# AcrylicShrimp/omok-ai

Measured on NVIDIA B200. Metric: mcts_simulations_per_sec, higher is better.
Workload: dtype f32

## Files before the change

### include/omok_b200.h

```cpp
#ifndef OMOK_B200_H
#define OMOK_B200_H

#include <stdint.h>

#ifdef __cplusplus
extern "C" {
#endif

#if defined(__GNUC__)
#define OMK_API __attribute__((visibility("default")))
#else
#define OMK_API
#endif

#define OMK_CELLS 81
#define OMK_NONE (-1)

enum {
    OMK_OK = 0,
    OMK_ERR_INVALID = -1,
    OMK_ERR_CUDA = -2,
    OMK_ERR_CAPACITY = -3,
    OMK_ERR_STATE = -4,
    OMK_ERR_NUMERIC = -5,
};

enum {
    OMK_EVAL_NET = 0,
    OMK_EVAL_HASH = 1,
};

enum { OMK_SAMPLE_BEST = 0, OMK_SAMPLE_BOLTZMANN = 1 };
enum { OMK_TURN_MODE_PLAYER = 0, OMK_TURN_MODE_OPPONENT = 1 };

typedef struct omk_ctx omk_ctx;

OMK_API const char *omk_last_error(void);
OMK_API int32_t omk_version(void);

OMK_API int32_t omk_ctx_create(int32_t device, int32_t capacity_envs, int32_t capacity_trees, int32_t capacity_nodes,
                       uint64_t seed, omk_ctx **out);
OMK_API int32_t omk_ctx_destroy(omk_ctx *ctx);
OMK_API int32_t omk_ctx_synchronize(omk_ctx *ctx);
OMK_API void *omk_ctx_stream(omk_ctx *ctx);
OMK_API int64_t omk_ctx_launch_count(omk_ctx *ctx);
OMK_API int32_t omk_ctx_transfer_bytes(omk_ctx *ctx, int64_t *out_h2d, int64_t *out_d2h);

#define OMK_NET_TENSORS 31
OMK_API int32_t omk_net_load_params(omk_ctx *ctx, const float *const *tensors, const int64_t *lens);
OMK_API int32_t omk_net_get_params(omk_ctx *ctx, float *const *tensors, const int64_t *lens);
OMK_API int32_t omk_net_init_random(omk_ctx *ctx, uint64_t seed);
OMK_API int32_t omk_net_eval(omk_ctx *ctx, const uint8_t *boards, const uint8_t *turns, int32_t n, int32_t mode,
                     float *out_p, float *out_v);
OMK_API int32_t omk_net_eval_images(omk_ctx *ctx, const float *images, int32_t n, float *out_p, float *out_v);

OMK_API int32_t omk_train_step(omk_ctx *ctx, const float *images, const float *pi, const float *z, int32_t n, float *out_losses);
OMK_API int32_t omk_train_backward(omk_ctx *ctx, const float *images, const float *pi, const float *z, int32_t n,
                           void **out_grads_device, int64_t *out_count);
OMK_API int32_t omk_train_apply(omk_ctx *ctx, float *out_losses);
OMK_API int32_t omk_train_get_grads(omk_ctx *ctx, float *const *tensors, const int64_t *lens);
OMK_API int32_t omk_train_reset_optimizer(omk_ctx *ctx);
OMK_API int32_t omk_train_comm_unique_id(omk_ctx *ctx, uint8_t *out_id);
OMK_API int32_t omk_train_comm_init(omk_ctx *ctx, const uint8_t *id, int32_t nranks, int32_t rank);
OMK_API int32_t omk_train_comm_destroy(omk_ctx *ctx);

OMK_API int32_t omk_debug_set_fc0_mode(omk_ctx *ctx, int32_t mode);
OMK_API int32_t omk_debug_set_tower_mode(omk_ctx *ctx, int32_t mode);
OMK_API int32_t omk_debug_set_fc0_chunk(omk_ctx *ctx, int32_t k_blocks);
OMK_API int32_t omk_debug_set_fc0_balance(omk_ctx *ctx, int32_t on);
OMK_API int32_t omk_debug_tower_timing(omk_ctx *ctx, int64_t *out64);
OMK_API int32_t omk_debug_get_buffer(omk_ctx *ctx, int32_t which, float *out, int64_t count);
OMK_API int32_t omk_debug_set_lane_min_trees(omk_ctx *ctx, int32_t min_trees);

OMK_API int32_t omk_env_reset(omk_ctx *ctx, const int32_t *ids, int32_t n);
OMK_API int32_t omk_env_step(omk_ctx *ctx, const int32_t *ids, const uint8_t *actions, int32_t n, int8_t *out_status,
                     uint32_t *out_legal);
OMK_API int32_t omk_env_step_device(omk_ctx *ctx, const uint8_t *actions_device, int32_t n, int8_t *out_status_device,
                            uint32_t *out_legal_device);
OMK_API int32_t omk_env_get(omk_ctx *ctx, const int32_t *ids, int32_t n, uint8_t *out_boards, uint8_t *out_turns,
                    uint16_t *out_legal_counts);
OMK_API int32_t omk_env_set(omk_ctx *ctx, const int32_t *ids, int32_t n, const uint8_t *boards, const uint8_t *turns);
OMK_API int32_t omk_env_encode(omk_ctx *ctx, const int32_t *ids, int32_t n, int32_t mode, float *out);
OMK_API int32_t omk_env_random_playout(omk_ctx *ctx, int32_t n, int32_t plies, uint8_t *out_actions, int8_t *out_status);

OMK_API int32_t omk_pool_new_games(omk_ctx *ctx, const int32_t *ids, int32_t n, const uint32_t *streams, int32_t evaluator);
OMK_API int32_t omk_pool_search(omk_ctx *ctx, const int32_t *ids, int32_t n, int32_t count, int32_t batch_size,
                        float epsilon, float alpha, int32_t evaluator);
OMK_API int32_t omk_search_set_virtual_loss(omk_ctx *ctx, int32_t enabled);
OMK_API int32_t omk_pool_sample(omk_ctx *ctx, const int32_t *ids, int32_t n, const uint8_t *modes,
                        const float *temperatures, int32_t *out_actions, float *out_policy);
OMK_API int32_t omk_pool_policy(omk_ctx *ctx, const int32_t *ids, int32_t n, float *out_policy, uint8_t *out_valid);
OMK_API int32_t omk_pool_ensure_action(omk_ctx *ctx, const int32_t *ids, const int32_t *actions, int32_t n,
                               int32_t evaluator);
OMK_API int32_t omk_pool_play(omk_ctx *ctx, const int32_t *ids, const int32_t *actions, int32_t n, int8_t *out_status);
OMK_API int32_t omk_pool_get_env(omk_ctx *ctx, int32_t id, uint8_t *out_board, uint8_t *out_turn,
                         uint16_t *out_legal_count);
OMK_API int32_t omk_pool_get_envs(omk_ctx *ctx, const int32_t *ids, int32_t n, uint8_t *out_boards, uint8_t *out_turns,
                          uint16_t *out_legal_counts, int8_t *out_status);
OMK_API int32_t omk_pool_root_stats(omk_ctx *ctx, int32_t id, uint64_t *out_n, float *out_w, float *out_p,
                            int32_t *out_status, float *out_policy);
OMK_API int32_t omk_pool_root_children(omk_ctx *ctx, int32_t id, int32_t *out_actions, uint64_t *out_n, float *out_w,
                               float *out_p, int32_t *out_len);
OMK_API int32_t omk_pool_tree_info(omk_ctx *ctx, int32_t id, int32_t *out_nodes, uint32_t *out_rng_counter);

enum {
    OMK_K_TOWER = 0,
    OMK_K_FC0 = 1,
    OMK_K_FC1 = 2,
    OMK_K_HEADS = 3,
    OMK_K_HASH = 4,
    OMK_K_SELECT = 5,
    OMK_K_APPLY = 6,
    OMK_K_MOVE = 7,
    OMK_K_COUNT = 8
};

typedef struct {
    int32_t n_games;
    int32_t count;
    int32_t batch_size;
    float epsilon;
    float alpha;
    float temperature;
    int32_t temperature_threshold;
    int32_t evaluator;
} omk_selfplay_config;

typedef struct {
    int64_t simulations;
    int64_t positions;
    int64_t nn_evals;
    int64_t games_finished;
    int64_t h2d_bytes, d2h_bytes;
    float gpu_ms;
    float kind_ms[OMK_K_COUNT];
    int64_t kind_launches[OMK_K_COUNT];
} omk_selfplay_stats;

OMK_API int32_t omk_selfplay_begin(omk_ctx *ctx, const omk_selfplay_config *cfg);
OMK_API int32_t omk_selfplay_run(omk_ctx *ctx, int32_t plies, int32_t profile, uint8_t *out_boards, float *out_policy,
                         int8_t *out_status, int32_t *out_actions, omk_selfplay_stats *stats);

OMK_API int32_t omk_replay_reset(omk_ctx *ctx, int64_t capacity);
OMK_API int32_t omk_replay_info(omk_ctx *ctx, int64_t *out_len, int64_t *out_rows_added, int64_t *out_episodes);
OMK_API int32_t omk_replay_get(omk_ctx *ctx, const int64_t *rows, int32_t n, uint8_t *out_boards, uint8_t *out_turns,
                       float *out_policy, float *out_z);
OMK_API int32_t omk_train_replay(omk_ctx *ctx, uint64_t seed, int64_t first_step, int32_t steps, int32_t n, float *out_losses,
                         int64_t *out_rows);

OMK_API int32_t omk_naive_move(omk_ctx *ctx, const uint8_t *boards, const uint8_t *turns, int32_t n, uint64_t seed,
                               const uint32_t *streams, int32_t *out_actions, uint8_t *out_forced);
OMK_API int32_t omk_eval_naive(omk_ctx *ctx, int32_t episodes, int32_t first_tree, int32_t count, int32_t batch_size, float epsilon,
                               float alpha, int32_t evaluator, uint64_t seed, int32_t *out_result, int8_t *out_moves,
                               int8_t *out_status, int64_t *out_stats, float *out_gpu_ms);

// ... 13 lines not shown
```

### omok-ai_b200/binding.py

```python
from __future__ import annotations

import ctypes as C
import os
import re

import numpy as np

CELLS = 81
NONE = -1
EVAL_NET, EVAL_HASH = 0, 1
SAMPLE_BEST, SAMPLE_BOLTZMANN = 0, 1

_HERE = os.path.dirname(os.path.abspath(__file__))
_ROOT = os.path.dirname(_HERE)

NET_LENS = [384, 128] + [4096, 32, 288, 1024, 32, 4096, 128] * 3 + [10368 * 512, 512, 512 * 512, 512, 512, 1, 512 * 81, 81]
NET_SHAPES = (
    [(1, 1, 3, 128), (128,)]
    + [(1, 1, 128, 32), (32,), (3, 3, 32, 1), (1, 1, 32, 32), (32,), (1, 1, 32, 128), (128,)] * 3
    + [(10368, 512), (512,), (512, 512), (512,), (512, 1), (1,), (512, 81), (81,)]
)


class OmkError(RuntimeError):
# ... 4 lines not shown

class SelfPlayConfig(C.Structure):
    _fields_ = [
        ("n_games", C.c_int32),
        ("count", C.c_int32),
        ("batch_size", C.c_int32),
        ("epsilon", C.c_float),
        ("alpha", C.c_float),
        ("temperature", C.c_float),
        ("temperature_threshold", C.c_int32),
        ("evaluator", C.c_int32),
    ]


class SelfPlayStats(C.Structure):
    _fields_ = [
        ("simulations", C.c_int64),
        ("positions", C.c_int64),
        ("nn_evals", C.c_int64),
        ("games_finished", C.c_int64),
        ("h2d_bytes", C.c_int64),
        ("d2h_bytes", C.c_int64),
        ("gpu_ms", C.c_float),
        ("kind_ms", C.c_float * 8),
        ("kind_launches", C.c_int64 * 8),
    ]

    KINDS = ("tower", "fc0", "fc1", "heads", "hash", "select_expand", "apply", "move")

    def by_kind(self):
        return {k: (float(self.kind_ms[i]), int(self.kind_launches[i])) for i, k in enumerate(self.KINDS)}


def lib_path() -> str:
    return os.path.join(_HERE, "libomok_b200.so")


def declared_symbols() -> list[str]:
    text = open(os.path.join(_ROOT, "include", "omok_b200.h")).read()
    return sorted(set(re.findall(r"OMK_API[^;(]*?\b(omk_\w+)\s*\(", text)))


_lib = None


def load_library():
    global _lib
    if _lib is not None:
        return _lib
    path = lib_path()
    if not os.path.exists(path):
        raise OmkError(-2, f"{path} is missing: run __graft_entry__.build() (there is no CPU fallback)")
    L = C.CDLL(path)
    P = C.POINTER
    i32, i64, u64, f32, vp = C.c_int32, C.c_int64, C.c_uint64, C.c_float, C.c_void_p
    L.omk_last_error.restype = C.c_char_p
    L.omk_version.restype = i32
    L.omk_ctx_create.argtypes = [i32, i32, i32, i32, u64, P(vp)]
    L.omk_ctx_destroy.argtypes = [vp]
    L.omk_ctx_synchronize.argtypes = [vp]
    L.omk_ctx_stream.argtypes = [vp]
    L.omk_ctx_stream.restype = vp
    L.omk_ctx_launch_count.argtypes = [vp]
    L.omk_ctx_launch_count.restype = i64
    L.omk_ctx_transfer_bytes.argtypes = [vp, P(i64), P(i64)]
    L.omk_net_load_params.argtypes = [vp, P(vp), P(i64)]
    L.omk_net_get_params.argtypes = [vp, P(vp), P(i64)]
    L.omk_net_init_random.argtypes = [vp, u64]
    L.omk_net_eval.argtypes = [vp, vp, vp, i32, i32, vp, vp]
    L.omk_net_eval_images.argtypes = [vp, vp, i32, vp, vp]
    L.omk_train_step.argtypes = [vp, vp, vp, vp, i32, vp]
    L.omk_train_backward.argtypes = [vp, vp, vp, vp, i32, P(vp), P(i64)]
    L.omk_train_apply.argtypes = [vp, vp]
    L.omk_train_get_grads.argtypes = [vp, P(vp), P(i64)]
    L.omk_train_reset_optimizer.argtypes = [vp]
    L.omk_train_comm_unique_id.argtypes = [vp, vp]
    L.omk_train_comm_init.argtypes = [vp, vp, i32, i32]
    L.omk_train_comm_destroy.argtypes = [vp]
    L.omk_debug_set_fc0_mode.argtypes = [vp, i32]
    L.omk_debug_set_tower_mode.argtypes = [vp, i32]
    L.omk_debug_set_fc0_chunk.argtypes = [vp, i32]
    L.omk_debug_set_fc0_balance.argtypes = [vp, i32]
    L.omk_debug_set_lane_min_trees.argtypes = [vp, i32]
    L.omk_debug_get_buffer.argtypes = [vp, i32, vp, i64]
    L.omk_debug_tower_timing.argtypes = [vp, vp]
    L.omk_env_reset.argtypes = [vp, vp, i32]
    L.omk_env_step.argtypes = [vp, vp, vp, i32, vp, vp]
    L.omk_env_step_device.argtypes = [vp, vp, i32, vp, vp]
    L.omk_env_get.argtypes = [vp, vp, i32, vp, vp, vp]
    L.omk_env_set.argtypes = [vp, vp, i32, vp, vp]
    L.omk_env_encode.argtypes = [vp, vp, i32, i32, vp]
    L.omk_env_random_playout.argtypes = [vp, i32, i32, vp, vp]
    L.omk_pool_new_games.argtypes = [vp, vp, i32, vp, i32]
    L.omk_pool_search.argtypes = [vp, vp, i32, i32, i32, f32, f32, i32]
    L.omk_search_set_virtual_loss.argtypes = [vp, i32]
    L.omk_pool_sample.argtypes = [vp, vp, i32, vp, vp, vp, vp]
    L.omk_pool_policy.argtypes = [vp, vp, i32, vp, vp]
    L.omk_pool_ensure_action.argtypes = [vp, vp, vp, i32, i32]
    L.omk_pool_play.argtypes = [vp, vp, vp, i32, vp]
    L.omk_pool_get_env.argtypes = [vp, i32, vp, vp, vp]
    L.omk_pool_get_envs.argtypes = [vp, vp, i32, vp, vp, vp, vp]
    L.omk_pool_root_stats.argtypes = [vp, i32, vp, vp, vp, vp, vp]
    L.omk_pool_root_children.argtypes = [vp, i32, vp, vp, vp, vp, vp]
    L.omk_pool_tree_info.argtypes = [vp, i32, vp, vp]
    L.omk_selfplay_begin.argtypes = [vp, P(SelfPlayConfig)]
    L.omk_selfplay_run.argtypes = [vp, i32, i32, vp, vp, vp, vp, P(SelfPlayStats)]
    L.omk_replay_reset.argtypes = [vp, i64]
    L.omk_replay_info.argtypes = [vp, P(i64), P(i64), P(i64)]
    L.omk_replay_get.argtypes = [vp, vp, i32, vp, vp, vp, vp]
    L.omk_train_replay.argtypes = [vp, u64, i64, i32, i32, vp, vp]
    L.omk_naive_move.argtypes = [vp, vp, vp, i32, u64, vp, vp, vp]
    L.omk_eval_naive.argtypes = [vp, i32, i32, i32, i32, f32, f32, i32, u64, vp, vp, vp, vp, P(f32)]
    L.omk_opponent_load_params.argtypes = [vp, P(vp), P(i64)]
    L.omk_opponent_from_net.argtypes = [vp]
    L.omk_opponent_eval.argtypes = [vp, vp, vp, i32, i32, vp, vp]
    L.omk_match.argtypes = [vp, i32, i32, i32, i32, f32, f32, i32, vp, vp, vp, vp, P(f32)]
    for name in declared_symbols():
        fn = getattr(L, name)
        if name not in ("omk_last_error", "omk_ctx_stream", "omk_ctx_launch_count"):
            fn.restype = i32
    _lib = L
    return L


def _ptr(a):
    return None if a is None else a.ctypes.data_as(C.c_void_p)


def _ids(ids):
    return None if ids is None else np.ascontiguousarray(ids, dtype=np.int32)


class Context:

    def __init__(self, device: int = 0, capacity_envs: int = 0, capacity_trees: int = 0, capacity_nodes: int = 4096,
                 seed: int = 0):
        self.L = load_library()
        h = C.c_void_p()
        self.h = None
        self._check(self.L.omk_ctx_create(device, capacity_envs, capacity_trees, capacity_nodes, seed, C.byref(h)))
        self.h = h
        self.capacity_envs, self.capacity_trees, self.capacity_nodes = capacity_envs, capacity_trees, capacity_nodes
        self.seed = seed

    def _check(self, rc: int):
        if rc != 0:
            raise OmkError(rc, self.L.omk_last_error().decode())

    def close(self):
        if self.h is not None:
            self.L.omk_ctx_destroy(self.h)
            self.h = None

    def __del__(self):
        try:
            self.close()
        except Exception:
            pass

    def synchronize(self):
        self._check(self.L.omk_ctx_synchronize(self.h))

    @property
    def stream(self) -> int:
        return int(self.L.omk_ctx_stream(self.h) or 0)

# ... 22 lines not shown

    def net_init_random(self, seed: int = 0):
        self._check(self.L.omk_net_init_random(self.h, seed))

    def net_eval(self, boards, turns, mode: int = 0, want_v: bool = True):
        boards = np.ascontiguousarray(boards, dtype=np.uint8).reshape(-1, CELLS)
        turns = np.ascontiguousarray(turns, dtype=np.uint8).reshape(-1)
        n = boards.shape[0]
        p = np.zeros((n, CELLS), dtype=np.float32)
        v = np.zeros(n, dtype=np.float32) if want_v else None
        self._check(self.L.omk_net_eval(self.h, _ptr(boards), _ptr(turns), n, mode, _ptr(p), _ptr(v)))
        return p, v

    def net_eval_images(self, images, want_v: bool = True):
        images = np.ascontiguousarray(images, dtype=np.float32).reshape(-1, 243)
        n = images.shape[0]
        p = np.zeros((n, CELLS), dtype=np.float32)
        v = np.zeros(n, dtype=np.float32) if want_v else None
        self._check(self.L.omk_net_eval_images(self.h, _ptr(images), n, _ptr(p), _ptr(v)))
        return p, v

    @staticmethod
    def _batch(images, pi, z):
        images = np.ascontiguousarray(images, dtype=np.float32).reshape(-1, 243)
        n = images.shape[0]
        pi = np.ascontiguousarray(pi, dtype=np.float32).reshape(n, CELLS)
        z = np.ascontiguousarray(z, dtype=np.float32).reshape(n)
        return images, pi, z, n

    def train_step(self, images, pi, z):
        images, pi, z, n = self._batch(images, pi, z)
        out = np.zeros(3, dtype=np.float32)
        self._check(self.L.omk_train_step(self.h, _ptr(images), _ptr(pi), _ptr(z), n, _ptr(out)))
        return float(out[0]), float(out[1]), float(out[2])

    def train_backward(self, images, pi, z):
        images, pi, z, n = self._batch(images, pi, z)
        ptr, cnt = C.c_void_p(), C.c_int64()
        self._check(self.L.omk_train_backward(self.h, _ptr(images), _ptr(pi), _ptr(z), n, C.byref(ptr), C.byref(cnt)))
        return int(ptr.value or 0), int(cnt.value)

    def train_apply(self):
        out = np.zeros(3, dtype=np.float32)
        self._check(self.L.omk_train_apply(self.h, _ptr(out)))
        return float(out[0]), float(out[1]), float(out[2])

    def train_get_grads(self):
        arrs = [np.zeros(n, dtype=np.float32) for n in NET_LENS]
        ptrs = (C.c_void_p * 31)(*[a.ctypes.data for a in arrs])
        lens = (C.c_int64 * 31)(*NET_LENS)
        self._check(self.L.omk_train_get_grads(self.h, ptrs, lens))
        return [a.reshape(s) for a, s in zip(arrs, NET_SHAPES)]

    def train_reset_optimizer(self):
        self._check(self.L.omk_train_reset_optimizer(self.h))

    def train_comm_unique_id(self) -> bytes:
        buf = np.zeros(128, dtype=np.uint8)
        self._check(self.L.omk_train_comm_unique_id(self.h, _ptr(buf)))
        return buf.tobytes()

    def train_comm_init(self, unique_id: bytes, nranks: int, rank: int):
        buf = np.frombuffer(unique_id, dtype=np.uint8).copy()
        self._check(self.L.omk_train_comm_init(self.h, _ptr(buf), nranks, rank))

    def train_comm_destroy(self):
        self._check(self.L.omk_train_comm_destroy(self.h))

    def debug_set_fc0_mode(self, mode: int):
        self._check(self.L.omk_debug_set_fc0_mode(self.h, mode))

    def debug_set_tower_mode(self, mode: int):
        self._check(self.L.omk_debug_set_tower_mode(self.h, mode))

    def debug_set_fc0_balance(self, on: bool):
        self._check(self.L.omk_debug_set_fc0_balance(self.h, 1 if on else 0))

    def debug_set_fc0_chunk(self, k_blocks: int):
        self._check(self.L.omk_debug_set_fc0_chunk(self.h, k_blocks))

    def debug_set_lane_min_trees(self, min_trees: int):
        self._check(self.L.omk_debug_set_lane_min_trees(self.h, min_trees))

    def debug_tower_timing(self):
        out = np.zeros(64, dtype=np.int64)
        self._check(self.L.omk_debug_tower_timing(self.h, _ptr(out)))
        return out

    def debug_get_buffer(self, which: int, count: int):
        out = np.zeros(count, dtype=np.float32)
        self._check(self.L.omk_debug_get_buffer(self.h, which, _ptr(out), count))
        return out

    def env_reset(self, ids=None, n=None):
        ids = _ids(ids)
        n = len(ids) if ids is not None else n
        self._check(self.L.omk_env_reset(self.h, _ptr(ids), n))

    def env_step(self, actions, ids=None, want_legal: bool = True):
        actions = np.ascontiguousarray(actions, dtype=np.uint8)
        ids = _ids(ids)
        n = actions.size
        status = np.zeros(n, dtype=np.int8)
        legal = np.zeros((n, 3), dtype=np.uint32) if want_legal else None
        self._check(self.L.omk_env_step(self.h, _ptr(ids), _ptr(actions), n, _ptr(status), _ptr(legal)))
        return status, legal

    def env_step_device(self, actions_dev: int, n: int, status_dev: int, legal_dev: int):
        self._check(self.L.omk_env_step_device(self.h, actions_dev, n, status_dev, legal_dev))

    def env_get(self, ids=None, n=None):
        ids = _ids(ids)
        n = len(ids) if ids is not None else n
        boards = np.zeros((n, CELLS), dtype=np.uint8)
        turns = np.zeros(n, dtype=np.uint8)
        legal = np.zeros(n, dtype=np.uint16)
        self._check(self.L.omk_env_get(self.h, _ptr(ids), n, _ptr(boards), _ptr(turns), _ptr(legal)))
        return boards, turns, legal

    def env_set(self, boards, turns, ids=None):
        boards = np.ascontiguousarray(boards, dtype=np.uint8).reshape(-1, CELLS)
        turns = np.ascontiguousarray(turns, dtype=np.uint8).reshape(-1)
        ids = _ids(ids)
        self._check(self.L.omk_env_set(self.h, _ptr(ids), boards.shape[0], _ptr(boards), _ptr(turns)))

    def env_encode(self, ids=None, n=None, mode: int = 0):
        ids = _ids(ids)
        n = len(ids) if ids is not None else n
        out = np.zeros((n, 243), dtype=np.float32)
        self._check(self.L.omk_env_encode(self.h, _ptr(ids), n, mode, _ptr(out)))
        return out

    def env_random_playout(self, n: int, plies: int, trace: bool = True):
        actions = np.zeros((plies, n), dtype=np.uint8) if trace else None
        status = np.zeros((plies, n), dtype=np.int8) if trace else None
        self._check(self.L.omk_env_random_playout(self.h, n, plies, _ptr(actions), _ptr(status)))
        return actions, status

    def pool_new_games(self, ids=None, n=None, streams=None, evaluator: int = EVAL_NET):
        ids = _ids(ids)
        n = len(ids) if ids is not None else n
        streams = None if streams is None else np.ascontiguousarray(streams, dtype=np.uint32)
        self._check(self.L.omk_pool_new_games(self.h, _ptr(ids), n, _ptr(streams), evaluator))

    def pool_search(self, ids=None, n=None, count=800, batch_size=16, epsilon=0.25, alpha=0.03, evaluator: int = EVAL_NET):
        ids = _ids(ids)
        n = len(ids) if ids is not None else n
        self._check(self.L.omk_pool_search(self.h, _ptr(ids), n, count, batch_size, epsilon, alpha, evaluator))

    def search_set_virtual_loss(self, enabled: bool):
        self._check(self.L.omk_search_set_virtual_loss(self.h, 1 if enabled else 0))

    def pool_sample(self, ids=None, n=None, modes=None, temperatures=None):
        ids = _ids(ids)
        n = len(ids) if ids is not None else n
        modes = None if modes is None else np.ascontiguousarray(modes, dtype=np.uint8)
        temperatures = None if temperatures is None else np.ascontiguousarray(temperatures, dtype=np.float32)
        actions = np.zeros(n, dtype=np.int32)
        policy = np.zeros((n, CELLS), dtype=np.float32)
        self._check(self.L.omk_pool_sample(self.h, _ptr(ids), n, _ptr(modes), _ptr(temperatures), _ptr(actions), _ptr(policy)))
        return actions, policy

    def pool_policy(self, ids=None, n=None):
        ids = _ids(ids)
        n = len(ids) if ids is not None else n
        policy = np.zeros((n, CELLS), dtype=np.float32)
# ... 156 lines not shown
```

### omok-ai_b200/csrc/fc_f16.cu

```cuda
#include <cstdio>
#include <cstdlib>
#include <cuda.h>

#include "omk_internal.h"
#include "tc_ptx.cuh"

namespace omk {

using namespace tc;

constexpr int F_BM = 128, F_BN = 256, F_BK = 64;
constexpr int F_N = 512;
constexpr int F_K0 = 10368, F_K1 = 512;
constexpr int F_A_BYTES = F_BM * F_BK * 2;
#ifndef OMK_F_CHUNK1
#define OMK_F_CHUNK1 1
#endif
#ifndef OMK_F_CHUNKH
#define OMK_F_CHUNKH 1
#endif
constexpr int F_SPLITK_KB = 9;
constexpr int F_CHUNK0 = 9, F_CHUNK0_FINE = 3;
constexpr int F_CHUNK1 = OMK_F_CHUNK1;
constexpr int F_CHUNKH = OMK_F_CHUNKH;
constexpr int kSplitKMaxRows = 2048;

struct FcBal {
    int full;
    int helpers;
    int m, tail;
    int mains;
    float4 *partial;
    uint32_t *flags;
};
constexpr int F_BAL_TAIL_MAX = 4;
constexpr size_t F_BAL_UNIT_F4 = 2 * 8 * 32 * 32;
__device__ __forceinline__ uint32_t ld_acquire_u32(const uint32_t *p) {
    uint32_t v;
    asm volatile("ld.acquire.gpu.global.u32 %0, [%1];" : "=r"(v) : "l"(p) : "memory");
    return v;
}

template <bool PAIR, int BN>
struct FcCfg {
    static constexpr int kStages = PAIR ? 3 : 2;
    static constexpr int kBRows = PAIR ? BN / 2 : BN;
    static constexpr int kBBytes = kBRows * F_BK * 2;
    static constexpr int kStageBytes = 2 * F_A_BYTES + 2 * kBBytes;
    static constexpr int kSmemBytes = kStages * kStageBytes + 1024 + 1024;
    static constexpr uint32_t kIdesc = idesc_f16(PAIR ? 256 : 128, BN);
    static constexpr int kDrainWarps = 4 * (BN / 128);
    static constexpr int kThreads = 64 + 32 * kDrainWarps;
    static constexpr uint32_t kTmemCols = 2 * BN;
};

template <int K, int CHUNK, bool PAIR, int BN = 256, bool HEADS = false, bool SPLITK = false>
__global__ void __launch_bounds__((FcCfg<PAIR, BN>::kThreads), 1)
    k_fc16(const __grid_constant__ CUtensorMap map_a_hi, const __grid_constant__ CUtensorMap map_a_lo,
           const __grid_constant__ CUtensorMap map_b_hi, const __grid_constant__ CUtensorMap map_b_lo,
           const float *__restrict__ bias, const float *__restrict__ inv_scale_p, float *__restrict__ C,
           __half *__restrict__ C_hi, __half *__restrict__ C_lo, const uint32_t *n_req, int max_rows,
           float *__restrict__ P_out = nullptr, float *__restrict__ V_out = nullptr, uint32_t *dev_error = nullptr,
           const FcBal bal = FcBal{}) {
    using Cfg = FcCfg<PAIR, BN>;
    static_assert(!HEADS || (BN == 128 && !PAIR), "the heads epilogue needs a whole logit row per thread");
    constexpr int CG = PAIR ? 2 : 1;
    static_assert(K % F_BK == 0 && (K / F_BK) % CHUNK == 0, "chunking must tile K");
    static_assert(!SPLITK || (!PAIR && !HEADS), "split-K is the one-CTA fc0 variant");
    constexpr int NKB = SPLITK ? F_SPLITK_KB : K / F_BK;
    static_assert(!SPLITK || (F_SPLITK_KB % CHUNK == 0 && (K / F_BK) % F_SPLITK_KB == 0), "split-K groups must tile K");
    constexpr int NCHUNK = NKB / CHUNK;
    const int kb_base = SPLITK ? (int)blockIdx.z * F_SPLITK_KB : 0;
    extern __shared__ uint8_t smem_raw[];
    const int rows = (int)min(*n_req, (uint32_t)max_rows);
    uint32_t rank = 0;
    int m0, n0;
    [[maybe_unused]] int role = 0, n_seq = NCHUNK, u0 = 0;
    [[maybe_unused]] int tile = 0;
    if constexpr (PAIR) {
        rank = cluster_rank();
        const int cid = blockIdx.x >> 1;
        tile = cid;
        if (cid >= bal.full && bal.helpers > 0) {
            if (cid < bal.full + bal.helpers) {
                role = 2;
                const int units = bal.mains * bal.tail, h = cid - bal.full;
                const int per = (units + bal.helpers - 1) / bal.helpers;
                u0 = h * per;
                n_seq = max(0, min(units, u0 + per) - u0);
            } else {
                role = 1;
                tile = cid - bal.helpers;
                n_seq = bal.m;
            }
        }
        const int pair = tile >> 1;
        m0 = pair * 256 + (int)rank * F_BM;
        n0 = (tile & 1) * BN;
        if (role != 2 && pair * 256 >= rows) return;
    } else {
        m0 = blockIdx.y * F_BM;
        n0 = blockIdx.x * BN;
        if (m0 >= rows) return;
    }
    const bool leader = rank == 0;

    const uint32_t base = (smem_u32(smem_raw) + 1023u) & ~1023u;
    const uint32_t bars = base + Cfg::kStages * Cfg::kStageBytes;
    const uint32_t full0 = bars, empty0 = bars + 8 * Cfg::kStages, tmem_full0 = bars + 16 * Cfg::kStages,
                   tmem_empty0 = tmem_full0 + 16, tmem_slot = tmem_empty0 + 16;
    const int warp = threadIdx.x >> 5, lane = threadIdx.x & 31;

    if (warp == 0 && lane == 0) {
        prefetch_map(&map_a_hi);
        prefetch_map(&map_a_lo);
        prefetch_map(&map_b_hi);
        prefetch_map(&map_b_lo);
        for (int s = 0; s < Cfg::kStages; ++s) {
            mbar_init(full0 + 8 * s, 1);
            mbar_init(empty0 + 8 * s, 1);
        }
        for (int b = 0; b < 2; ++b) {
            mbar_init(tmem_full0 + 8 * b, 1);
            mbar_init(tmem_empty0 + 8 * b, (PAIR ? 2 : 1) * Cfg::kDrainWarps);
        }
        mbar_fence_init();
    }
    if (warp == 1) tmem_alloc<CG>(tmem_slot, Cfg::kTmemCols);
    fence_before();
    __syncthreads();
    if constexpr (PAIR) cluster_sync_all();
    fence_after();
    uint32_t tmem_base;
    asm volatile("ld.shared.u32 %0, [%1];" : "=r"(tmem_base) : "r"(tmem_slot));

    if (warp == 0) {
        if (lane == 0) {
            if constexpr (PAIR) {
                int it = 0;
                for (int i = 0; i < n_seq; ++i) {
                    int ch = i, mm = m0, nn = n0;
                    if (role == 2) {
                        const int u = u0 + i, tl = bal.full + u / bal.tail;
                        ch = bal.m + u % bal.tail;
                        mm = (tl >> 1) * 256 + (int)rank * F_BM;
                        nn = (tl & 1) * BN;
                        if ((tl >> 1) * 256 >= rows) continue;
                    }
                    for (int kc = 0; kc < CHUNK; ++kc, ++it) {
                        const int kb = ch * CHUNK + kc, s = it % Cfg::kStages;
                        const uint32_t ph = (uint32_t)(it / Cfg::kStages) & 1u;
                        mbar_wait(empty0 + 8 * s, ph ^ 1u);
                        const uint32_t st = base + s * Cfg::kStageBytes;
                        const uint32_t lbar = mapa(full0 + 8 * s, 0);
                        if (leader) mbar_expect_tx(full0 + 8 * s, 2 * Cfg::kStageBytes);
                        tma_load_2d_2sm(st, &map_a_hi, lbar, kb * F_BK, mm);
                        tma_load_2d_2sm(st + F_A_BYTES, &map_a_lo, lbar, kb * F_BK, mm);
                        tma_load_2d_2sm(st + 2 * F_A_BYTES, &map_b_hi, lbar, kb * F_BK, nn + (int)rank * 128);
                        tma_load_2d_2sm(st + 2 * F_A_BYTES + Cfg::kBBytes, &map_b_lo, lbar, kb * F_BK, nn + (int)rank * 128);
                    }
                }
            }
            for (int kb = 0; kb < (PAIR ? 0 : NKB); ++kb) {
                const int s = kb % Cfg::kStages;
                const uint32_t ph = (uint32_t)(kb / Cfg::kStages) & 1u;
                mbar_wait(empty0 + 8 * s, ph ^ 1u);
                const uint32_t st = base + s * Cfg::kStageBytes;
                if constexpr (PAIR) {
                } else {
                    const uint32_t bar = full0 + 8 * s;
                    mbar_expect_tx(bar, Cfg::kStageBytes);
                    tma_load_2d(st, &map_a_hi, bar, (kb_base + kb) * F_BK, m0);
                    tma_load_2d(st + F_A_BYTES, &map_a_lo, bar, (kb_base + kb) * F_BK, m0);
                    tma_load_2d(st + 2 * F_A_BYTES, &map_b_hi, bar, (kb_base + kb) * F_BK, n0);
                    tma_load_2d(st + 2 * F_A_BYTES + Cfg::kBBytes, &map_b_lo, bar, (kb_base + kb) * F_BK, n0);
                }
            }
        }
    } else if (warp == 1) {
        if (leader && lane == 0) {
            for (int i = 0, ci = 0, it = 0; i < n_seq; ++i) {
                if constexpr (PAIR) {
                    if (role == 2 && ((bal.full + (u0 + i) / bal.tail) >> 1) * 256 >= rows) continue;
                }
                const int buf = ci & 1;
                const uint32_t use = (uint32_t)(ci >> 1);
                ++ci;
                mbar_wait(tmem_empty0 + 8 * buf, (use & 1u) ^ 1u);
                fence_after();
                const uint32_t tmem_acc = tmem_base + (uint32_t)(buf * BN);
                for (int kc = 0; kc < CHUNK; ++kc, ++it) {
                    const int s = it % Cfg::kStages;
                    const uint32_t ph = (uint32_t)(it / Cfg::kStages) & 1u;
                    mbar_wait(full0 + 8 * s, ph);
                    fence_after();
                    const uint32_t st = base + s * Cfg::kStageBytes;
                    const uint64_t a_hi = desc_sw128(st), a_lo = desc_sw128(st + F_A_BYTES);
                    const uint64_t b_hi = desc_sw128(st + 2 * F_A_BYTES), b_lo = desc_sw128(st + 2 * F_A_BYTES + Cfg::kBBytes);
#pragma unroll
                    for (int k = 0; k < F_BK / 16; ++k) {
                        const uint64_t adv = (uint64_t)((k * 32) >> 4);
                        umma_f16_ss<CG>(tmem_acc, a_lo + adv, b_hi + adv, Cfg::kIdesc, (kc | k) != 0 ? 1u : 0u);
                        umma_f16_ss<CG>(tmem_acc, a_hi + adv, b_lo + adv, Cfg::kIdesc, 1u);
                        umma_f16_ss<CG>(tmem_acc, a_hi + adv, b_hi + adv, Cfg::kIdesc, 1u);
                    }
                    if constexpr (PAIR) umma_commit_2sm(empty0 + 8 * s); else umma_commit(empty0 + 8 * s);
                }
                if constexpr (PAIR) umma_commit_2sm(tmem_full0 + 8 * buf); else umma_commit(tmem_full0 + 8 * buf);
            }
        }
    } else {
        const int q = warp & 3, half = (warp - 2) >> 2;
        float acc[128];
#pragma unroll
        for (int j = 0; j < 128; ++j) acc[j] = 0.0f;
        for (int ch = 0, ci = 0; ch < n_seq; ++ch) {
            [[maybe_unused]] float4 *unit_dst = nullptr;
            [[maybe_unused]] int unit_main = 0;
            if constexpr (PAIR) {
                if (role == 2) {
                    const int u = u0 + ch;
                    unit_main = u / bal.tail;
                    if (((bal.full + unit_main) >> 1) * 256 >= rows) continue;
                    unit_dst = bal.partial + (((size_t)u * 2 + rank) * 8 + (size_t)(warp - 2)) * 1024 + lane;
                }
            }
            const int buf = ci & 1;
            const uint32_t use = (uint32_t)(ci >> 1);
            ++ci;
            mbar_wait(tmem_full0 + 8 * buf, use & 1u);
            fence_after();
#pragma unroll
            for (int c = 0; c < 128; c += 32) {
                float v[32];
                tmem_ld32(tmem_base + ((uint32_t)(q * 32) << 16) + (uint32_t)(buf * BN + half * 128 + c), v);
                tmem_wait_ld();
                if (PAIR && role == 2) {
#pragma unroll
                    for (int j = 0; j < 32; j += 4) unit_dst[(size_t)((c + j) >> 2) * 32] = make_float4(v[j], v[j + 1], v[j + 2], v[j + 3]);
                } else {
#pragma unroll
                    for (int j = 0; j < 32; ++j) acc[c + j] += v[j];
                }
            }
            fence_before();
            __syncwarp();
            if (lane == 0) {
                if constexpr (PAIR) mbar_arrive_cluster(mapa(tmem_empty0 + 8 * buf, 0)); else mbar_arrive(tmem_empty0 + 8 * buf);
            }
            if constexpr (PAIR) {
                if (role == 2) {
                    __threadfence();
                    __syncwarp();
                    if (lane == 0) atomicAdd(bal.flags + unit_main, 1u);
                }
            }
            if constexpr (SPLITK) {
                const int prow = m0 + q * 32 + lane;
// ... 21 lines not shown
                    for (int c4 = 0; c4 < 32; ++c4) {
                        const float4 v = __ldcg(src + (size_t)c4 * 32);
                        acc[4 * c4 + 0] += v.x; acc[4 * c4 + 1] += v.y; acc[4 * c4 + 2] += v.z; acc[4 * c4 + 3] += v.w;
                    }
                }
                __syncwarp();
                if (lane == 0 && atomicAdd(bal.flags + 128 + k, 1u) == 15u) {
                    atomicExch(bal.flags + k, 0u);
                    atomicExch(bal.flags + 128 + k, 0u);
                }
            }
        }
        const int row = m0 + q * 32 + lane;
        const size_t coff = (size_t)row * F_N + n0 + half * 128;
        const float *brow = bias + n0 + half * 128;
        const float inv_scale = *inv_scale_p;
        if constexpr (SPLITK) {
        } else if constexpr (HEADS) {
            if (row < rows) {
                float mx = -INFINITY;
#pragma unroll
                for (int j = 0; j < kCells; ++j) {
                    acc[j] = fmaf(acc[j], inv_scale, brow[j]);
                    mx = fmaxf(mx, acc[j]);
                }
                float sum = 0.0f;
#pragma unroll
                for (int j = 0; j < kCells; ++j) {
                    acc[j] = expf(acc[j] - mx);
                    sum += acc[j];
                }
                const float inv = 1.0f / sum;
                const float vlogit = fmaf(acc[kCells], inv_scale, brow[kCells]);
                if (!(sum >= 1.0f && sum < INFINITY) || !(fabsf(vlogit) < INFINITY)) atomicOr(dev_error, 2u);
                float *prow = P_out + (size_t)row * kRow;
#pragma unroll
                for (int j = 0; j < 80; j += 4)
                    *reinterpret_cast<float4 *>(prow + j) = make_float4(acc[j] * inv, acc[j + 1] * inv, acc[j + 2] * inv, acc[j + 3] * inv);
                prow[80] = acc[80] * inv;
                V_out[row] = tanhf(vlogit);
            }
        } else if (row < rows && role != 2) {
#pragma unroll
            for (int j = 0; j < 128; j += 8) {
                float o[8];
#pragma unroll
                for (int i = 0; i < 8; i += 4) {
                    const float4 b = *reinterpret_cast<const float4 *>(brow + j + i);
                    o[i + 0] = fmaf(acc[j + i + 0], inv_scale, b.x);
                    o[i + 1] = fmaf(acc[j + i + 1], inv_scale, b.y);
                    o[i + 2] = fmaf(acc[j + i + 2], inv_scale, b.z);
                    o[i + 3] = fmaf(acc[j + i + 3], inv_scale, b.w);
                }
#pragma unroll
                for (int i = 0; i < 8; ++i) o[i] = fmaxf(o[i], 0.2f * o[i]);
                if (C) {
                    *reinterpret_cast<float4 *>(C + coff + j) = make_float4(o[0], o[1], o[2], o[3]);
                    *reinterpret_cast<float4 *>(C + coff + j + 4) = make_float4(o[4], o[5], o[6], o[7]);
                }
                if (C_hi) {
                    uint4 h, l;
                    split2_f16(o[0], o[1], h.x, l.x);
                    split2_f16(o[2], o[3], h.y, l.y);
                    split2_f16(o[4], o[5], h.z, l.z);
                    split2_f16(o[6], o[7], h.w, l.w);
                    *reinterpret_cast<uint4 *>(C_hi + coff + j) = h;
                    *reinterpret_cast<uint4 *>(C_lo + coff + j) = l;
                }
            }
        }
    }
    fence_before();
    __syncthreads();
    if constexpr (PAIR) cluster_sync_all();
    if (warp == 1) {
        fence_after();
        tmem_dealloc<CG>(tmem_base, Cfg::kTmemCols);
    }
}

__global__ void k_fc0_reduce(const float *__restrict__ partial, int nchunks, int ws_rows, const float *__restrict__ bias,
                             const float *__restrict__ inv_scale_p, __half *__restrict__ C_hi, __half *__restrict__ C_lo,
                             const uint32_t *n_req, int max_rows) {
    const int rows = (int)min(*n_req, (uint32_t)max_rows);
    const int idx = blockIdx.x * blockDim.x + threadIdx.x;
    const int row = idx >> 6, j = (idx & 63) * 8;
    if (row >= rows) return;
    float acc[8];
#pragma unroll
    for (int i = 0; i < 8; ++i) acc[i] = 0.0f;
    for (int z0 = 0; z0 < nchunks; z0 += 6) {
        float4 a[6], b[6];
#pragma unroll
        for (int i = 0; i < 6; ++i) {
            const int z = min(z0 + i, nchunks - 1);
            const float *p = partial + ((size_t)z * ws_rows + row) * F_N + j;
            a[i] = *reinterpret_cast<const float4 *>(p);
            b[i] = *reinterpret_cast<const float4 *>(p + 4);
        }
#pragma unroll
        for (int i = 0; i < 6; ++i) {
            if (z0 + i >= nchunks) break;
            acc[0] += a[i].x; acc[1] += a[i].y; acc[2] += a[i].z; acc[3] += a[i].w;
            acc[4] += b[i].x; acc[5] += b[i].y; acc[6] += b[i].z; acc[7] += b[i].w;
        }
    }
    const float inv_scale = *inv_scale_p;
    float o[8];
#pragma unroll
    for (int i = 0; i < 8; ++i) {
        o[i] = fmaf(acc[i], inv_scale, bias[j + i]);
        o[i] = fmaxf(o[i], 0.2f * o[i]);
    }
    uint4 h, l;
    split2_f16(o[0], o[1], h.x, l.x);
    split2_f16(o[2], o[3], h.y, l.y);
    split2_f16(o[4], o[5], h.z, l.z);
    split2_f16(o[6], o[7], h.w, l.w);
    *reinterpret_cast<uint4 *>(C_hi + (size_t)row * F_N + j) = h;
    *reinterpret_cast<uint4 *>(C_lo + (size_t)row * F_N + j) = l;
}

__global__ void k_absmax_bits(const float *__restrict__ w, long long n, uint32_t *out) {
    uint32_t m = 0;
    for (long long i = (long long)blockIdx.x * blockDim.x + threadIdx.x; i < n; i += (long long)gridDim.x * blockDim.x)
        m = max(m, __float_as_uint(w[i]) & 0x7FFFFFFFu);
#pragma unroll
    for (int off = 16; off > 0; off >>= 1) m = max(m, __shfl_xor_sync(0xffffffffu, m, off));
    if ((threadIdx.x & 31) == 0 && m) atomicMax(out, m);
}

__global__ void k_fc16_split_weights(const float *__restrict__ W, const uint32_t *absmax_bits, __half *__restrict__ hi,
                                     __half *__restrict__ lo, float *inv_scale, int K, int N) {
    __shared__ float tile[32][33];
    const float scale = f16_split_scale(*absmax_bits);
    if (blockIdx.x == 0 && blockIdx.y == 0 && threadIdx.x == 0) *inv_scale = 1.0f / scale;
    const int k0 = blockIdx.x * 32, n0 = blockIdx.y * 32;
    const int tx = threadIdx.x & 31, ty = threadIdx.x >> 5;
    for (int r = ty; r < 32; r += 8) tile[r][tx] = W[(size_t)(k0 + r) * N + n0 + tx];
    __syncthreads();
    for (int r = ty; r < 32; r += 8) {
        const float x = tile[tx][r] * scale;
        const __half h = __float2half_rn(x);
        hi[(size_t)(n0 + r) * K + k0 + tx] = h;
        lo[(size_t)(n0 + r) * K + k0 + tx] = __float2half_rn(x - __half2float(h));
    }
}

__global__ void k_f32_to_split16(const float *__restrict__ x, __half *__restrict__ hi, __half *__restrict__ lo, long long n) {
    for (long long i = (long long)blockIdx.x * blockDim.x + threadIdx.x; i < n; i += (long long)gridDim.x * blockDim.x) {
        const __half h = __float2half_rn(x[i]);
        hi[i] = h;
        lo[i] = __float2half_rn(x[i] - __half2float(h));
    }
}
__global__ void k_split16_to_f32(const __half *__restrict__ hi, const __half *__restrict__ lo, float *__restrict__ x, long long n) {
    for (long long i = (long long)blockIdx.x * blockDim.x + threadIdx.x; i < n; i += (long long)gridDim.x * blockDim.x)
        x[i] = __half2float(hi[i]) + __half2float(lo[i]);
}
void launch_f32_to_split16(omk_ctx *c, const float *x, __half *hi, __half *lo, long long n) {
    k_f32_to_split16<<<1184, 256, 0, c->stream>>>(x, hi, lo, n);
    c->launches++;
}
void launch_split16_to_f32(omk_ctx *c, const __half *hi, const __half *lo, float *x, long long n) {
    k_split16_to_f32<<<1184, 256, 0, c->stream>>>(hi, lo, x, n);
    c->launches++;
// ... 32 lines not shown
    const cuuint32_t box[3] = {32, 32, 1};
    const cuuint32_t estr[3] = {1, 1, 1};
    return fn(map, CU_TENSOR_MAP_DATA_TYPE_FLOAT16, 3, ptr, dims, strides, box, estr, CU_TENSOR_MAP_INTERLEAVE_NONE,
              CU_TENSOR_MAP_SWIZZLE_64B, CU_TENSOR_MAP_L2_PROMOTION_NONE, CU_TENSOR_MAP_FLOAT_OOB_FILL_NONE) == CUDA_SUCCESS;
}

struct Fc16State {
    int pair_slots = 0;
};
void Fc16StateFree::operator()(Fc16State *s) const { delete s; }

static Fc16State *state16_of(omk_ctx *c) {
    if (!c->fc16_state) c->fc16_state.reset(new Fc16State());
    return c->fc16_state.get();
}

bool fc16_prepare_weights(omk_ctx *c) {
    NetWeights &w = *c->model;
    if (!w.fc0_wt_h16) {
        FcImages f;
        if (f.fc0_wt_h16.alloc((size_t)F_K0 * F_N) != cudaSuccess || f.fc0_wt_l16.alloc((size_t)F_K0 * F_N) != cudaSuccess ||
            f.fc1_wt_h16.alloc((size_t)F_K1 * F_N) != cudaSuccess || f.fc1_wt_l16.alloc((size_t)F_K1 * F_N) != cudaSuccess ||
            f.heads_wt_h16.alloc((size_t)F_K1 * 128) != cudaSuccess || f.heads_wt_l16.alloc((size_t)F_K1 * 128) != cudaSuccess ||
            f.fc_inv_scale.alloc(3) != cudaSuccess || f.fc_absmax.alloc(3) != cudaSuccess)
            return false;
        static_cast<FcImages &>(w) = std::move(f);
    }
    cudaMemsetAsync(w.fc_absmax, 0, sizeof(uint32_t) * 3, c->stream);
    k_absmax_bits<<<592, 256, 0, c->stream>>>(w.t[23], (long long)F_K0 * F_N, w.fc_absmax);
    k_absmax_bits<<<148, 256, 0, c->stream>>>(w.t[25], (long long)F_K1 * F_N, w.fc_absmax + 1);
    k_absmax_bits<<<64, 256, 0, c->stream>>>(w.heads_w, (long long)F_K1 * 128, w.fc_absmax + 2);
    k_fc16_split_weights<<<dim3(F_K0 / 32, F_N / 32), 256, 0, c->stream>>>(w.t[23], w.fc_absmax, w.fc0_wt_h16, w.fc0_wt_l16,
                                                                           w.fc_inv_scale, F_K0, F_N);
    k_fc16_split_weights<<<dim3(F_K1 / 32, F_N / 32), 256, 0, c->stream>>>(w.t[25], w.fc_absmax + 1, w.fc1_wt_h16, w.fc1_wt_l16,
                                                                           w.fc_inv_scale + 1, F_K1, F_N);
    k_fc16_split_weights<<<dim3(F_K1 / 32, 128 / 32), 256, 0, c->stream>>>(w.heads_w, w.fc_absmax + 2, w.heads_wt_h16, w.heads_wt_l16,
                                                                         w.fc_inv_scale + 2, F_K1, 128);
    c->launches += 6;
    if (!encode_map16(&w.map0_b_hi, w.fc0_wt_h16, F_N, 128, F_K0)) return false;
    if (!encode_map16(&w.map0_b_lo, w.fc0_wt_l16, F_N, 128, F_K0)) return false;
    if (!encode_map16(&w.map0s_b_hi, w.fc0_wt_h16, F_N, F_BN, F_K0)) return false;
    if (!encode_map16(&w.map0s_b_lo, w.fc0_wt_l16, F_N, F_BN, F_K0)) return false;
    if (!encode_map16(&w.map1_b_hi, w.fc1_wt_h16, F_N, F_BN, F_K1)) return false;
    if (!encode_map16(&w.map1_b_lo, w.fc1_wt_l16, F_N, F_BN, F_K1)) return false;
    if (!encode_map16(&w.map2_b_hi, w.heads_wt_h16, 128, 128, F_K1)) return false;
    if (!encode_map16(&w.map2_b_lo, w.heads_wt_l16, 128, 128, F_K1)) return false;
    w.weights_ready = true;
    return true;
}

bool fc16_encode_act_maps(Activations &a) {
    ActMaps &m = a.maps;
    const uint64_t rows = (uint64_t)a.act_rows;
    return encode_map16(&m.map0_a_hi, a.act0_h16, rows, F_BM, F_K0) && encode_map16(&m.map0_a_lo, a.act0_l16, rows, F_BM, F_K0) &&
           encode_map16(&m.map1_a_hi, a.act1_h16, rows, F_BM, F_K1) && encode_map16(&m.map1_a_lo, a.act1_l16, rows, F_BM, F_K1) &&
           encode_map16(&m.map2_a_hi, a.act2_h16, rows, F_BM, F_K1) && encode_map16(&m.map2_a_lo, a.act2_l16, rows, F_BM, F_K1) &&
           encode_map_tower_store(&m.tower_st_hi, a.act0_h16, rows) && encode_map_tower_store(&m.tower_st_lo, a.act0_l16, rows);
}

static bool check_launch(const char *what) {
    const cudaError_t le = cudaPeekAtLastError();
    if (le == cudaSuccess) return true;
    fprintf(stderr, "omok_b200: %s launch failed: %s\n", what, cudaGetErrorString(le));
    return false;
}

bool launch_fc0_f16(omk_ctx *c, int rows_bound) {
    const NetWeights &m = *c->model;
    const ActMaps *am = m.weights_ready ? &c->ws.maps : nullptr;
    if (!am) return false;
    const bool fine = c->fc0_chunk == F_CHUNK0_FINE;
    static const int splitk_env = getenv("OMK_FC0_SPLITK_MAX") ? atoi(getenv("OMK_FC0_SPLITK_MAX")) : -1;
    const int splitk_max = splitk_env >= 0 ? splitk_env : (fine ? 1024 : kSplitKMaxRows);
    if (rows_bound <= splitk_max) {
        const int kChunks = F_K0 / F_BK / (fine ? F_CHUNK0_FINE : F_CHUNK0);
        const int mt = (rows_bound + F_BM - 1) / F_BM, ws_rows = mt * F_BM;
        if (c->ws.splitk_partial.grow(c->stream, (size_t)kChunks * ws_rows * F_N) != cudaSuccess) return false;
        float *partial = c->ws.splitk_partial;
        static const int narrow_env = getenv("OMK_FC0_SPLITK_NARROW") ? atoi(getenv("OMK_FC0_SPLITK_NARROW")) : -1;
        if (mt <= (narrow_env >= 0 ? narrow_env : 2)) {
            using Cfg = FcCfg<false, 128>;
            auto sk = fine ? k_fc16<F_K0, F_CHUNK0_FINE, false, 128, false, true> : k_fc16<F_K0, F_CHUNK0, false, 128, false, true>;
            cudaFuncSetAttribute(sk, cudaFuncAttributeMaxDynamicSharedMemorySize, Cfg::kSmemBytes);
            sk<<<dim3(F_N / 128, mt, F_K0 / F_BK / F_SPLITK_KB), Cfg::kThreads, Cfg::kSmemBytes, c->stream>>>(
                am->map0_a_hi, am->map0_a_lo, m.map0_b_hi, m.map0_b_lo, m.t[24], m.fc_inv_scale, partial, nullptr,
                nullptr, c->ws.n_req, rows_bound, nullptr, nullptr, nullptr, FcBal{});
        } else {
            using Cfg = FcCfg<false, 256>;
            auto sk = fine ? k_fc16<F_K0, F_CHUNK0_FINE, false, 256, false, true> : k_fc16<F_K0, F_CHUNK0, false, 256, false, true>;
            cudaFuncSetAttribute(sk, cudaFuncAttributeMaxDynamicSharedMemorySize, Cfg::kSmemBytes);
            sk<<<dim3(F_N / F_BN, mt, F_K0 / F_BK / F_SPLITK_KB), Cfg::kThreads, Cfg::kSmemBytes, c->stream>>>(
                am->map0_a_hi, am->map0_a_lo, m.map0s_b_hi, m.map0s_b_lo, m.t[24], m.fc_inv_scale, partial, nullptr,
                nullptr, c->ws.n_req, rows_bound, nullptr, nullptr, nullptr, FcBal{});
        }
        k_fc0_reduce<<<(rows_bound * 64 + 255) / 256, 256, 0, c->stream>>>(partial, kChunks, ws_rows, m.t[24],
                                                                            m.fc_inv_scale, c->ws.act1_h16, c->ws.act1_l16,
                                                                            c->ws.n_req, rows_bound);
        c->launches += 2;
        return check_launch("fc0 (fp16 split, split-K)");
    }
    auto kern = fine ? k_fc16<F_K0, F_CHUNK0_FINE, true> : k_fc16<F_K0, F_CHUNK0, true>;
    cudaFuncSetAttribute(kern, cudaFuncAttributeMaxDynamicSharedMemorySize, FcCfg<true, 256>::kSmemBytes);
    const int pairs = (rows_bound + 255) / 256;
    cudaLaunchConfig_t cfg{};
    cfg.gridDim = dim3(2 * (F_N / F_BN) * pairs, 1);
    cfg.blockDim = dim3(FcCfg<true, 256>::kThreads);
    cfg.dynamicSmemBytes = FcCfg<true, 256>::kSmemBytes;
    cfg.stream = c->stream;
    cudaLaunchAttribute attr[1];
    attr[0].id = cudaLaunchAttributeClusterDimension;
    attr[0].val.clusterDim.x = 2;
    attr[0].val.clusterDim.y = 1;
    attr[0].val.clusterDim.z = 1;
    cfg.attrs = attr;
    cfg.numAttrs = 1;
    const float *bias_p = m.t[24];
    const float *inv_p = m.fc_inv_scale;
    float *c_f32 = nullptr;
    __half *c_hi = c->ws.act1_h16, *c_lo = c->ws.act1_l16;
    const uint32_t *nreq_p = c->ws.n_req;
    float *no_p = nullptr, *no_v = nullptr;
    uint32_t *no_err = nullptr;
    FcBal bal{};
    if (!fine && c->fc0_balance) {
        Fc16State *st = state16_of(c);
        if (st->pair_slots == 0) {
            int n = 0;
            if (cudaOccupancyMaxActiveClusters(&n, kern, &cfg) != cudaSuccess) { cudaGetLastError(); n = 0; }
            st->pair_slots = n > 0 ? n : -1;
        }
        const int P = st->pair_slots, T = (F_N / F_BN) * pairs, NC = F_K0 / F_BK / F_CHUNK0;
        const int R = P > 0 ? T % P : 0, H = P - R;
        if (R > 0 && R <= 128 && H > 0) {
            int tail = 0;
            for (int t = 1; t <= F_BAL_TAIL_MAX; ++t)
                if ((R * t + H - 1) / H + 1 <= NC - t) tail = t;
            if (tail > 0) {
                const int units = R * tail;
                bool ok = true;
                Workspace &w = c->ws;
                if (!w.bal_flags)
                    ok = w.bal_flags.alloc(256) == cudaSuccess && cudaMemsetAsync(w.bal_flags, 0, w.bal_flags.bytes(), c->stream) == cudaSuccess;
                if (!ok || w.bal_partial.grow(c->stream, F_BAL_UNIT_F4 * (size_t)units) != cudaSuccess) return false;
                bal.full = T - R;
                bal.helpers = H;
                bal.mains = R;
                bal.tail = tail;
                bal.m = NC - tail;
                bal.partial = w.bal_partial;
                bal.flags = w.bal_flags;
                cfg.gridDim = dim3(2 * (T + H), 1);
            }
        }
    }
    const cudaError_t e = cudaLaunchKernelEx(&cfg, kern, am->map0_a_hi, am->map0_a_lo, m.map0_b_hi, m.map0_b_lo, bias_p, inv_p, c_f32,
                                             c_hi, c_lo, nreq_p, rows_bound, no_p, no_v, no_err, bal);
    if (e != cudaSuccess) fprintf(stderr, "omok_b200: cudaLaunchKernelEx(k_fc16 pair): %s\n", cudaGetErrorString(e));
    c->launches++;
    return e == cudaSuccess && check_launch("fc0 (fp16 split)");
}

bool launch_fc1_f16(omk_ctx *c, int rows_bound) {
    const NetWeights &m = *c->model;
    const ActMaps *am = m.weights_ready ? &c->ws.maps : nullptr;
    if (!am) return false;
    using Cfg = FcCfg<false, 256>;
    auto kern = k_fc16<F_K1, F_CHUNK1, false>;
    cudaFuncSetAttribute(kern, cudaFuncAttributeMaxDynamicSharedMemorySize, Cfg::kSmemBytes);
    const int mt = (rows_bound + F_BM - 1) / F_BM;
    kern<<<dim3(F_N / F_BN, mt), Cfg::kThreads, Cfg::kSmemBytes, c->stream>>>(
        am->map1_a_hi, am->map1_a_lo, m.map1_b_hi, m.map1_b_lo, m.t[26], m.fc_inv_scale + 1, nullptr, c->ws.act2_h16,
        c->ws.act2_l16, c->ws.n_req, rows_bound, nullptr, nullptr, nullptr, FcBal{});
    c->launches++;
    return check_launch("fc1 (fp16 split)");
}

bool launch_heads_f16(omk_ctx *c, int rows_bound) {
    const NetWeights &m = *c->model;
    const ActMaps *am = m.weights_ready ? &c->ws.maps : nullptr;
    if (!am) return false;
    using Cfg = FcCfg<false, 128>;
    auto kern = k_fc16<F_K1, F_CHUNKH, false, 128, true>;
    cudaFuncSetAttribute(kern, cudaFuncAttributeMaxDynamicSharedMemorySize, Cfg::kSmemBytes);
    const int mt = (rows_bound + F_BM - 1) / F_BM;
    kern<<<dim3(1, mt), Cfg::kThreads, Cfg::kSmemBytes, c->stream>>>(
        am->map2_a_hi, am->map2_a_lo, m.map2_b_hi, m.map2_b_lo, m.heads_b, m.fc_inv_scale + 2, nullptr, nullptr, nullptr,
        c->ws.n_req, rows_bound, c->ws.P, c->ws.V, c->dev_error, FcBal{});
    c->launches++;
    return check_launch("heads (fp16 split)");
}

}
```

### omok-ai_b200/csrc/omk_api.cu

```cuda
#include <cstdio>
#include <cstdlib>
#include <cstring>
#include <string>
#include <vector>

#include <utility>

#include "omk_internal.h"

using namespace omk;

static thread_local std::string g_err;
static int32_t fail(int32_t code, const std::string &msg) {
    g_err = msg;
    return code;
}
#define CK(call)                                                                                        \
    do {                                                                                                \
        cudaError_t e__ = (call);                                                                       \
        if (e__ != cudaSuccess)                                                                         \
            return fail(OMK_ERR_CUDA, std::string(#call) + ": " + cudaGetErrorString(e__));             \
    } while (0)
#define CKV(call)                                                                                       \
    do {                                                                                                \
// ... 471 lines not shown
extern "C" int32_t omk_train_apply(omk_ctx *c, float *out_losses) {
    CK(cudaSetDevice(c->device));
    if (c->train_n < 1) return fail(OMK_ERR_STATE, "omk_train_backward has not produced a gradient");
    if (const char *e = train_apply_step(c)) return fail(OMK_ERR_CUDA, std::string("omk_train_apply: ") + e);
    c->net_pack_dirty = true;
    float l[3] = {0, 0, 0};
    if (const char *e = train_report_losses(c, c->train_n, l)) return fail(OMK_ERR_CUDA, std::string("omk_train_apply: ") + e);
    c->train_n = 0;
    if (!(l[2] == l[2]) || l[2] > 3.0e38f) return fail(OMK_ERR_NUMERIC, "the training loss is not finite");
    if (out_losses) memcpy(out_losses, l, sizeof l);
    return OMK_OK;
}

extern "C" int32_t omk_train_step(omk_ctx *c, const float *images, const float *pi, const float *z, int32_t n, float *out_losses) {
    int32_t rc = train_backward_impl(c, images, pi, z, n, nullptr, nullptr, false);
    if (rc) return rc;
    return omk_train_apply(c, out_losses);
}

extern "C" int32_t omk_train_get_grads(omk_ctx *c, float *const *tensors, const int64_t *lens) {
    CK(cudaSetDevice(c->device));
    const float *g = train_grad_buffer(c);
    if (!g) return fail(OMK_ERR_STATE, "omk_train_backward has not run");
    long long off = 0;
    for (int i = 0; i < kNetTensors; ++i) {
        if (!tensors[i] || lens[i] != kLens[i]) return fail(OMK_ERR_INVALID, "bad tensor length");
        CK(copy_d2h(c, tensors[i], g + off, sizeof(float) * (size_t)kLens[i], c->stream));
        off += kLens[i];
    }
    CK(cudaStreamSynchronize(c->stream));
    return OMK_OK;
}

extern "C" int32_t omk_train_reset_optimizer(omk_ctx *c) {
    CK(cudaSetDevice(c->device));
    train_reset_optimizer(c);
    CK(cudaStreamSynchronize(c->stream));
    return OMK_OK;
}

extern "C" int32_t omk_train_comm_unique_id(omk_ctx *c, uint8_t *out_id) {
    if (!out_id) return fail(OMK_ERR_INVALID, "out_id is NULL");
    if (const char *e = train_comm_unique_id(c, out_id)) return fail(OMK_ERR_STATE, std::string("NCCL: ") + e);
    return OMK_OK;
}
extern "C" int32_t omk_train_comm_init(omk_ctx *c, const uint8_t *id, int32_t nranks, int32_t rank) {
    CK(cudaSetDevice(c->device));
    if (!id || nranks < 1 || rank < 0 || rank >= nranks) return fail(OMK_ERR_INVALID, "bad communicator arguments");
    if (const char *e = train_comm_init(c, id, nranks, rank)) return fail(OMK_ERR_STATE, std::string("NCCL: ") + e);
    return OMK_OK;
}
extern "C" int32_t omk_train_comm_destroy(omk_ctx *c) {
    CK(cudaSetDevice(c->device));
    train_comm_destroy(c);
    return OMK_OK;
}

extern "C" int32_t omk_debug_set_fc0_mode(omk_ctx *c, int32_t mode) {
    if (mode != 0 && mode != 1) return fail(OMK_ERR_INVALID, "fc0 mode must be 1 (tcgen05 3xFP16) or 0 (fp32 CUDA cores, A/B check)");
    c->fc0_mode = mode;
    return OMK_OK;
}
extern "C" int32_t omk_debug_set_tower_mode(omk_ctx *c, int32_t mode) {
    if (mode != 0 && mode != 1) return fail(OMK_ERR_INVALID, "tower mode must be 1 (tcgen05 3xFP16) or 0 (fp32 CUDA cores, A/B check)");
    c->tower_mode = mode;
    return OMK_OK;
}
extern "C" int32_t omk_debug_set_fc0_balance(omk_ctx *c, int32_t on) {
    if (on != 0 && on != 1) return fail(OMK_ERR_INVALID, "fc0 balance must be 0 or 1");
    c->fc0_balance = on;
    return OMK_OK;
}
extern "C" int32_t omk_debug_set_fc0_chunk(omk_ctx *c, int32_t k_blocks) {
    if (k_blocks != 3 && k_blocks != 9) return fail(OMK_ERR_INVALID, "fc0 chunk must be 9 (default) or 3 (finer accumulation)");
    CK(cudaStreamSynchronize(c->stream));
    c->fc0_chunk = k_blocks;
    return OMK_OK;
}
extern "C" int32_t omk_debug_set_lane_min_trees(omk_ctx *c, int32_t min_trees) {
    if (min_trees < 0) return fail(OMK_ERR_INVALID, "min_trees < 0");
    c->lane_min_trees = min_trees;
    return OMK_OK;
}
extern "C" int32_t omk_debug_tower_timing(omk_ctx *c, int64_t *out64) {
    CK(cudaSetDevice(c->device));
    CK(cudaStreamSynchronize(c->stream));
    tower16_read_timing(reinterpret_cast<long long *>(out64));
    return OMK_OK;
}
extern "C" int32_t omk_debug_get_buffer(omk_ctx *c, int32_t which, float *out, int64_t count) {
    CK(cudaSetDevice(c->device));
    if (which >= 8 && which <= 10) {
        if (!out || count < 0) return fail(OMK_ERR_INVALID, "bad buffer");
        const __half *hi = which == 8 ? c->ws.act0_h16 : which == 9 ? c->ws.act1_h16 : c->ws.act2_h16;
        const __half *lo = which == 8 ? c->ws.act0_l16 : which == 9 ? c->ws.act1_l16 : c->ws.act2_l16;
        if (!hi || !lo) return fail(OMK_ERR_STATE, "the tensor-core activation buffers do not exist yet (no network call so far)");
        float *tmp = nullptr;
        SCRATCH(0, (size_t)(count > 0 ? count : 1), tmp);
        launch_split16_to_f32(c, hi, lo, tmp, count);
        CK(copy_d2h(c, out, tmp, sizeof(float) * (size_t)count, c->stream));
        CK(cudaStreamSynchronize(c->stream));
        return OMK_OK;
    }
    const float *src = which == 0 ? c->ws.act0 : which == 1 ? c->ws.act1 : which == 2 ? c->ws.act2 : which == 3 ? c->ws.logits.get() : nullptr;
    if (!src || !out || count < 0) return fail(OMK_ERR_INVALID, "bad buffer id");
    CK(copy_d2h(c, out, src, sizeof(float) * (size_t)count, c->stream));
    CK(cudaStreamSynchronize(c->stream));
    return OMK_OK;
}

extern "C" int32_t omk_env_reset(omk_ctx *c, const int32_t *ids, int32_t n) {
    CK(cudaSetDevice(c->device));
    const int32_t *d_ids;
    int32_t rc = stage_ids(c, ids, n, &d_ids, c->cap_envs);
    if (rc) return rc;
    launch_env_reset(c, d_ids, n);
    CK(cudaStreamSynchronize(c->stream));
    return OMK_OK;
}

extern "C" int32_t omk_env_step(omk_ctx *c, const int32_t *ids, const uint8_t *actions, int32_t n, int8_t *out_status,
                                uint32_t *out_legal) {
    CK(cudaSetDevice(c->device));
    if (!actions) return fail(OMK_ERR_INVALID, "actions is NULL");
    const int32_t *d_ids;
    int32_t rc = stage_ids(c, ids, n, &d_ids, c->cap_envs);
    if (rc) return rc;
    if (n == 0) return OMK_OK;
    uint8_t *d_act = nullptr;
    int8_t *d_st = nullptr;
    uint32_t *d_legal = nullptr;
    SCRATCH(0, (size_t)n, d_act);
    SCRATCH(1, (size_t)n, d_st);
    if (out_legal) SCRATCH(2, 3 * (size_t)n, d_legal);
    CK(copy_h2d(c, d_act, actions, (size_t)n, c->stream));
    launch_env_step(c, d_ids, d_act, n, d_st, d_legal);
    if (out_status) CK(copy_d2h(c, out_status, d_st, (size_t)n, c->stream));
    if (out_legal) CK(copy_d2h(c, out_legal, d_legal, sizeof(uint32_t) * 3 * (size_t)n, c->stream));
    CK(cudaStreamSynchronize(c->stream));
    CK(cudaGetLastError());
    return OMK_OK;
}

extern "C" int32_t omk_env_step_device(omk_ctx *c, const uint8_t *actions_device, int32_t n, int8_t *out_status_device,
                                       uint32_t *out_legal_device) {
    if (n < 0 || n > c->cap_envs) return fail(OMK_ERR_INVALID, "n exceeds capacity_envs");
    launch_env_step(c, nullptr, actions_device, n, out_status_device, out_legal_device);
    return OMK_OK;
}

extern "C" int32_t omk_env_get(omk_ctx *c, const int32_t *ids, int32_t n, uint8_t *out_boards, uint8_t *out_turns,
                               uint16_t *out_legal_counts) {
    CK(cudaSetDevice(c->device));
    const int32_t *d_ids;
    int32_t rc = stage_ids(c, ids, n, &d_ids, c->cap_envs);
    if (rc) return rc;
    if (n == 0) return OMK_OK;
    uint8_t *d_b = nullptr, *d_t = nullptr;
    uint16_t *d_l = nullptr;
    SCRATCH(0, (size_t)n * kCells, d_b);
    SCRATCH(1, (size_t)n, d_t);
    SCRATCH(2, (size_t)n, d_l);
    launch_env_get(c, d_ids, n, d_b, d_t, d_l);
    if (out_boards) CK(copy_d2h(c, out_boards, d_b, (size_t)n * kCells, c->stream));
    if (out_turns) CK(copy_d2h(c, out_turns, d_t, (size_t)n, c->stream));
    if (out_legal_counts) CK(copy_d2h(c, out_legal_counts, d_l, sizeof(uint16_t) * (size_t)n, c->stream));
// ... 1009 lines not shown
```

### omok-ai_b200/csrc/omk_internal.h

```cpp
#pragma once
#include <cstdint>
#include <memory>
#include <utility>
#include <vector>
#include <cuda.h>
#include <cuda_fp16.h>
#include <cuda_runtime.h>

#include "../../include/omok_b200.h"
#include "omk_device.cuh"

namespace omk {

constexpr int kMaxBatchPerTree = 64;
constexpr int kNetTensors = 31;

enum ApplyMode { kApplySearch = 0, kApplyNewGame = 1, kApplyEnsure = 2 };

struct DeviceMem {
    static cudaError_t alloc(void **p, size_t bytes) { return cudaMalloc(p, bytes); }
    static void release(void *p) { cudaFree(p); }
};
struct PinnedMem {
    static cudaError_t alloc(void **p, size_t bytes) { return cudaHostAlloc(p, bytes, cudaHostAllocDefault); }
// ... 115 lines not shown
    uint8_t *turns;
    float *pi;
    float *z;
    long long cap;
};
struct ReplayStore {
    Buf<uint8_t> boards, turns;
    Buf<float> pi, z;
    long long cap = 0;
    ReplayRing view() const { return {boards, turns, pi, z, cap}; }
};
struct ReplayCounters {
    long long added, len, episodes;
    uint32_t done, pad;
};
struct ReplayStaging {
    int games = 0;
    Buf<uint8_t> boards;
    Buf<float> pi;
    Buf<int32_t> len;
};
struct Replay {
    ReplayStore ring;
    Buf<ReplayCounters> counters;
    long long added = 0, len = 0, episodes = 0;
    ReplayStaging stage;
    cudaStream_t stream = nullptr;
    cudaEvent_t ev_commit = nullptr;
};

struct Fc16State;
struct TrainState;
struct Fc16StateFree { void operator()(Fc16State *s) const; };
struct TrainStateFree { void operator()(TrainState *t) const; };

}

struct omk_prof_span {
    cudaEvent_t a, b;
    int kind;
};

struct omk_ctx {
    ~omk_ctx();
    int device = 0;
    int prof_level = 0;
    std::vector<omk_prof_span> prof_spans;
    std::vector<cudaEvent_t> prof_pool;
    int n_sms = 0;
    int cap_envs = 0, cap_trees = 0, cap_nodes = 0;
    uint64_t seed = 0;
    cudaStream_t stream = nullptr;
    int64_t launches = 0;
    int64_t h2d_bytes = 0, d2h_bytes = 0;
    cudaStream_t lane1_stream = nullptr;
    omk::Workspace lane1_ws;
    cudaEvent_t lane_fork = nullptr, lane_join = nullptr;
    int lane_min_trees = 768;
    omk::Buf<uint8_t> scratch[3];
    std::vector<uint8_t> id_seen;
    int id_base = 0;

    omk::Buf<omk::EnvRec> envs;
    omk::Buf<omk::TreeHdr> tree_hdrs;
    omk::Buf<uint8_t> tree_nodes;
    omk::Buf<uint16_t> remap;
    omk::Buf<uint32_t> dev_error;
    omk::Buf<unsigned long long> dev_sims;

    omk::NetWeights net;
    omk::NetWeights opp;
    omk::NetWeights *model = &net;
    omk::Workspace ws;
    int virtual_loss = 0;
    int fc0_balance = 0;
    int fc0_chunk = 9;
    int fc0_mode = 1;
    std::unique_ptr<omk::Fc16State, omk::Fc16StateFree> fc16_state;
    int tower16_pairs = 0;
    std::unique_ptr<omk::TrainState, omk::TrainStateFree> train_state;
    int train_n = 0;
    bool net_pack_dirty = false;
    int tower_mode = 1;

    omk_selfplay_config sp_cfg{};
    bool sp_active = false;
    omk::Buf<int32_t> sp_ply;
    omk::Buf<uint8_t> sp_buf;
    static constexpr int kSpRing = 4;
    omk::Buf<uint8_t> sp_ring_dev;
    omk::PinnedBuf<uint8_t> sp_ring_host;
    size_t sp_ring_slot_bytes = 0;
    cudaStream_t sp_copy_stream = nullptr;
    cudaEvent_t sp_ev_rec[kSpRing][2] = {}, sp_ev_copy[kSpRing] = {};
    omk::Replay rp;
    omk::Buf<uint8_t> eval_buf;
    cudaEvent_t ev0 = nullptr, ev1 = nullptr;
};

namespace omk {

void launch_env_reset(omk_ctx *c, const int32_t *ids_dev, int n);
void launch_env_step(omk_ctx *c, const int32_t *ids_dev, const uint8_t *actions_dev, int n, int8_t *status_dev,
                     uint32_t *legal_dev);
void launch_env_get(omk_ctx *c, const int32_t *ids_dev, int n, uint8_t *boards_dev, uint8_t *turns_dev,
                    uint16_t *legal_dev);
void launch_env_set(omk_ctx *c, const int32_t *ids_dev, int n, const uint8_t *boards_dev, const uint8_t *turns_dev);
void launch_env_encode(omk_ctx *c, const int32_t *ids_dev, int n, int mode, float *out_dev);
void launch_env_playout(omk_ctx *c, int n, int plies, uint8_t *actions_dev, int8_t *status_dev);
void launch_pack_boards(omk_ctx *c, const uint8_t *boards_dev, const uint8_t *turns_dev, int n, int mode);

void launch_new_games(omk_ctx *c, const int32_t *ids_dev, int n, const uint32_t *streams_dev,
                      const int8_t *only_if_terminal, const float *root_policy);
void launch_root_noise(omk_ctx *c, const int32_t *ids_dev, int n, float epsilon, float alpha);
void launch_select_expand(omk_ctx *c, const int32_t *ids_dev, int n, int batch);
void launch_apply(omk_ctx *c, const int32_t *ids_dev, int n, int mode);
void launch_sample(omk_ctx *c, const int32_t *ids_dev, int n, const uint8_t *modes_dev, const float *temps_dev,
                   int32_t *actions_dev, float *policy_dev, uint8_t *valid_dev);
void launch_ensure_prepare(omk_ctx *c, const int32_t *ids_dev, const int32_t *actions_dev, int n);
void launch_play(omk_ctx *c, const int32_t *ids_dev, const int32_t *actions_dev, int n, int8_t *status_dev);
void launch_root_children(omk_ctx *c, int tree, int32_t *actions_dev, unsigned long long *n_dev, float *w_dev,
                          float *p_dev, int32_t *len_dev, float *policy_dev, uint32_t *misc_dev);
void launch_eval_hash(omk_ctx *c, int rows_bound);
void launch_pool_get_envs(omk_ctx *c, const int32_t *ids_dev, int n, uint8_t *boards_dev, uint8_t *turns_dev,
                          uint16_t *legal_dev, int8_t *status_dev);
void launch_reset_requests(omk_ctx *c);
void launch_sp_prepare(omk_ctx *c, int g0, int n, int32_t *mover, int32_t *other, uint8_t *modes, float *temps);
void launch_sp_record(omk_ctx *c, int n, const int32_t *mover, const int32_t *actions, const float *policy_in,
                      uint8_t *boards_out, float *policy_out, int32_t *actions_out);
void launch_sp_advance(omk_ctx *c, int g0, int n, const int8_t *status, unsigned long long *counters);

void launch_rp_stage(omk_ctx *c, int g0, int n, const uint8_t *boards, const float *policy);
void launch_rp_commit(omk_ctx *c, int n, const int8_t *status);
void launch_rp_sample(omk_ctx *c, uint64_t seed, long long first_step, int steps, long long len, int m, int64_t *rows);
void launch_rp_gather(omk_ctx *c, const int64_t *rows, int m, float *img, float *pi, float *z);
void launch_rp_get(omk_ctx *c, const int64_t *rows, int n, uint8_t *boards, uint8_t *turns, float *pi, float *z);

void launch_naive_move_boards(omk_ctx *c, const uint8_t *boards, const uint8_t *turns, const uint32_t *streams, int n, uint64_t key,
                              int32_t *actions, uint8_t *forced);
void launch_naive_move_trees(omk_ctx *c, const int32_t *ids, int n, int first_tree, const int32_t *ply, uint64_t key, int32_t *actions);
void launch_eval_init(omk_ctx *c, int episodes, int first_tree, int32_t *ids, int32_t *ply, int8_t *moves, int8_t *final_status,
                      int32_t *counters);
void launch_eval_advance(omk_ctx *c, int32_t *ids, int n, const int32_t *actions, const int8_t *status, int first_tree, int32_t *ply,
                         int8_t *moves, int8_t *final_status, int32_t *counters);
void launch_match_init(omk_ctx *c, int pairs, int first_tree, int32_t *ids, uint32_t *streams, int8_t *moves, int8_t *final_status,
                       int32_t *counters);
void launch_match_advance(omk_ctx *c, int pairs, int first_tree, int half, const int *live, int32_t *ids, int32_t *actions,
                          const int8_t *status, const int8_t *other_status, int8_t *moves, int8_t *final_status, int32_t *counters);

bool prof_begin(omk_ctx *c, int kind, int min_level);
void prof_end(omk_ctx *c, bool opened);

bool net_forward(omk_ctx *c, const float *images_dev , int max_rows);
void net_pack_heads(omk_ctx *c);
void launch_net_init_random(omk_ctx *c, uint64_t seed);

bool ensure_activations(omk_ctx *c, int rows);

bool fc16_prepare_weights(omk_ctx *c);
bool launch_fc0_f16(omk_ctx *c, int rows_bound);
bool launch_fc1_f16(omk_ctx *c, int rows_bound);
bool launch_heads_f16(omk_ctx *c, int rows_bound);
bool fc16_encode_act_maps(Activations &a);
void launch_f32_to_split16(omk_ctx *c, const float *x, __half *hi, __half *lo, long long n);
void launch_split16_to_f32(omk_ctx *c, const __half *hi, const __half *lo, float *x, long long n);

const char *train_backward_step(omk_ctx *c, const float *images, const float *pi, const float *z, int n, float **grads_dev);
const char *train_apply_step(omk_ctx *c);
const char *train_report_losses(omk_ctx *c, int n, float *out3);
const char *train_minibatch_buffers(omk_ctx *c, int n, float **img, float **pi, float **z);
const char *train_backward_resident(omk_ctx *c, int n);
const char *train_report_losses_device(omk_ctx *c, int n, float *dst3);
float *train_grad_buffer(omk_ctx *c);
void train_reset_optimizer(omk_ctx *c);
const char *train_comm_unique_id(omk_ctx *c, uint8_t *out128);
const char *train_comm_init(omk_ctx *c, const uint8_t *id128, int nranks, int rank);
const char *train_comm_destroy(omk_ctx *c);

bool tower16_prepare_weights(omk_ctx *c);
bool launch_tower_f16(omk_ctx *c, const float *images_dev, int rows_bound);
void tower16_read_timing(long long *out64);

}
// ... 1 lines not shown
```

### omok-ai_b200/csrc/tc_ptx.cuh

```cuda
#pragma once
#include <cstdint>
#include <cuda_fp16.h>
#include <cuda.h>
#include <cuda_runtime.h>

namespace omk {
namespace tc {

__device__ __forceinline__ uint32_t smem_u32(const void *p) { return (uint32_t)__cvta_generic_to_shared(p); }

__device__ __forceinline__ void mbar_init(uint32_t bar, uint32_t count) {
    asm volatile("mbarrier.init.shared::cta.b64 [%0], %1;" ::"r"(bar), "r"(count));
}
__device__ __forceinline__ void mbar_fence_init() { asm volatile("fence.mbarrier_init.release.cluster;" ::: "memory"); }
__device__ __forceinline__ void mbar_expect_tx(uint32_t bar, uint32_t bytes) {
    asm volatile("mbarrier.arrive.expect_tx.shared::cta.b64 _, [%0], %1;" ::"r"(bar), "r"(bytes) : "memory");
}
__device__ __forceinline__ void mbar_arrive(uint32_t bar) {
    asm volatile("mbarrier.arrive.shared::cta.b64 _, [%0];" ::"r"(bar) : "memory");
}
__device__ __forceinline__ void mbar_arrive_cluster(uint32_t cluster_bar) {
    asm volatile("mbarrier.arrive.release.cluster.shared::cluster.b64 _, [%0];" ::"r"(cluster_bar) : "memory");
}
__device__ __forceinline__ void mbar_arrive_cluster_relaxed(uint32_t cluster_bar) {
    asm volatile("mbarrier.arrive.relaxed.cluster.shared::cluster.b64 _, [%0];" ::"r"(cluster_bar) : "memory");
}
__device__ __forceinline__ void mbar_wait(uint32_t bar, uint32_t parity) {
    uint32_t done = 0;
    for (uint32_t spin = 0; spin < (1u << 24); ++spin) {
        asm volatile(
            "{\n\t.reg .pred p;\n\t"
            "mbarrier.try_wait.parity.shared::cta.b64 p, [%1], %2;\n\t"
            "selp.u32 %0, 1, 0, p;\n\t}"
            : "=r"(done)
            : "r"(bar), "r"(parity)
            : "memory");
        if (done) return;
    }
    __trap();
}

__device__ __forceinline__ bool elect_one() {
    uint32_t pred;
    asm volatile("{\n\t.reg .pred p;\n\telect.sync _|p, 0xffffffff;\n\tselp.u32 %0, 1, 0, p;\n\t}" : "=r"(pred));
    return pred != 0;
}

__device__ __forceinline__ uint32_t cluster_rank() {
    uint32_t r;
    asm volatile("mov.u32 %0, %%cluster_ctarank;" : "=r"(r));
    return r;
}
__device__ __forceinline__ uint32_t mapa(uint32_t addr, uint32_t rank) {
    uint32_t r;
    asm volatile("mapa.shared::cluster.u32 %0, %1, %2;" : "=r"(r) : "r"(addr), "r"(rank));
    return r;
}
__device__ __forceinline__ void cluster_arrive() { asm volatile("barrier.cluster.arrive.release.aligned;" ::: "memory"); }
__device__ __forceinline__ void cluster_wait() { asm volatile("barrier.cluster.wait.acquire.aligned;" ::: "memory"); }
__device__ __forceinline__ void cluster_sync_all() {
    cluster_arrive();
    cluster_wait();
}

__device__ __forceinline__ void bulk_load(uint32_t dst, const void *src, uint32_t bytes, uint32_t bar) {
    asm volatile("cp.async.bulk.shared::cluster.global.mbarrier::complete_tx::bytes [%0], [%1], %2, [%3];"
                 ::"r"(dst), "l"(src), "r"(bytes), "r"(bar)
                 : "memory");
}
__device__ __forceinline__ void tma_load_2d(uint32_t dst, const void *map, uint32_t bar, int c0, int c1) {
    asm volatile(
        "cp.async.bulk.tensor.2d.shared::cluster.global.mbarrier::complete_tx::bytes [%0], [%1, {%3, %4}], [%2];"
        ::"r"(dst), "l"(map), "r"(bar), "r"(c0), "r"(c1)
        : "memory");
}
__device__ __forceinline__ void tma_load_2d_2sm(uint32_t dst, const void *map, uint32_t leader_bar, int c0, int c1) {
    asm volatile(
        "cp.async.bulk.tensor.2d.cta_group::2.shared::cluster.global.mbarrier::complete_tx::bytes [%0], [%1, {%3, %4}], [%2];"
        ::"r"(dst), "l"(map), "r"(leader_bar), "r"(c0), "r"(c1)
        : "memory");
}
__device__ __forceinline__ void tma_store_3d(const void *map, uint32_t src, int c0, int c1, int c2) {
    asm volatile("cp.async.bulk.tensor.3d.global.shared::cta.bulk_group [%0, {%2, %3, %4}], [%1];"
                 ::"l"(map), "r"(src), "r"(c0), "r"(c1), "r"(c2)
                 : "memory");
}
__device__ __forceinline__ void bulk_commit() { asm volatile("cp.async.bulk.commit_group;" ::: "memory"); }
__device__ __forceinline__ void bulk_wait_read0() { asm volatile("cp.async.bulk.wait_group.read 0;" ::: "memory"); }
__device__ __forceinline__ void bulk_wait_all0() { asm volatile("cp.async.bulk.wait_group 0;" ::: "memory"); }
__device__ __forceinline__ void sts128(uint32_t addr, const uint4 &v) {
    asm volatile("st.shared.v4.b32 [%0], {%1, %2, %3, %4};" ::"r"(addr), "r"(v.x), "r"(v.y), "r"(v.z), "r"(v.w) : "memory");
}
__device__ __forceinline__ void prefetch_map(const void *map) { asm volatile("prefetch.tensormap [%0];" ::"l"(map)); }
__device__ __forceinline__ void fence_proxy_async_smem() { asm volatile("fence.proxy.async.shared::cta;" ::: "memory"); }

__device__ __forceinline__ uint64_t desc_sw128(uint32_t saddr) {
    return (uint64_t)((saddr & 0x3FFFF) >> 4) | ((uint64_t)(1024 >> 4) << 32) | ((uint64_t)1 << 46) | ((uint64_t)2 << 61);
}
__device__ __forceinline__ uint64_t desc_nosw(uint32_t saddr, uint32_t lbo, uint32_t sbo) {
    return (uint64_t)((saddr & 0x3FFFF) >> 4) | ((uint64_t)((lbo >> 4) & 0x3FFF) << 16) | ((uint64_t)((sbo >> 4) & 0x3FFF) << 32) | ((uint64_t)1 << 46);
}
__host__ __device__ constexpr uint32_t idesc_f16(uint32_t M, uint32_t N) { return (1u << 4) | ((N >> 3) << 17) | ((M >> 4) << 24); }

template <int CG>
__device__ __forceinline__ void tmem_alloc(uint32_t slot_saddr, uint32_t cols) {
    if constexpr (CG == 1) {
        asm volatile("tcgen05.alloc.cta_group::1.sync.aligned.shared::cta.b32 [%0], %1;" ::"r"(slot_saddr), "r"(cols) : "memory");
        asm volatile("tcgen05.relinquish_alloc_permit.cta_group::1.sync.aligned;" ::: "memory");
    } else {
        asm volatile("tcgen05.alloc.cta_group::2.sync.aligned.shared::cta.b32 [%0], %1;" ::"r"(slot_saddr), "r"(cols) : "memory");
        asm volatile("tcgen05.relinquish_alloc_permit.cta_group::2.sync.aligned;" ::: "memory");
    }
}
template <int CG>
__device__ __forceinline__ void tmem_dealloc(uint32_t taddr, uint32_t cols) {
    if constexpr (CG == 1)
        asm volatile("tcgen05.dealloc.cta_group::1.sync.aligned.b32 %0, %1;" ::"r"(taddr), "r"(cols) : "memory");
    else
        asm volatile("tcgen05.dealloc.cta_group::2.sync.aligned.b32 %0, %1;" ::"r"(taddr), "r"(cols) : "memory");
}
__device__ __forceinline__ void fence_before() { asm volatile("tcgen05.fence::before_thread_sync;" ::: "memory"); }
__device__ __forceinline__ void fence_after() { asm volatile("tcgen05.fence::after_thread_sync;" ::: "memory"); }

template <int CG>
__device__ __forceinline__ void umma_f16_ss(uint32_t tmem_d, uint64_t da, uint64_t db, uint32_t idesc, uint32_t accumulate) {
    if constexpr (CG == 1)
        asm volatile(
            "{\n\t.reg .pred p;\n\tsetp.ne.b32 p, %4, 0;\n\t"
            "tcgen05.mma.cta_group::1.kind::f16 [%0], %1, %2, %3, p;\n\t}"
            ::"r"(tmem_d), "l"(da), "l"(db), "r"(idesc), "r"(accumulate)
            : "memory");
    else
        asm volatile(
            "{\n\t.reg .pred p;\n\tsetp.ne.b32 p, %4, 0;\n\t"
            "tcgen05.mma.cta_group::2.kind::f16 [%0], %1, %2, %3, p;\n\t}"
            ::"r"(tmem_d), "l"(da), "l"(db), "r"(idesc), "r"(accumulate)
            : "memory");
}
__device__ __forceinline__ void umma_f16_ts(uint32_t tmem_d, uint32_t tmem_a, uint64_t db, uint32_t idesc, uint32_t accumulate) {
    asm volatile(
        "{\n\t.reg .pred p;\n\tsetp.ne.b32 p, %4, 0;\n\t"
        "tcgen05.mma.cta_group::1.kind::f16 [%0], [%1], %2, %3, p;\n\t}"
        ::"r"(tmem_d), "r"(tmem_a), "l"(db), "r"(idesc), "r"(accumulate)
        : "memory");
}
__device__ __forceinline__ void umma_commit(uint32_t bar) {
// ... 63 lines not shown
```

### omok-ai_b200/csrc/tower_f16.cu

```cuda
#include <cstdio>
#include <cstdlib>

#include "omk_internal.h"
#include "tc_ptx.cuh"

namespace omk {

using namespace tc;

constexpr int T16_THREADS = 256;
constexpr uint32_t T16_TMEM_COLS = 256;
constexpr uint32_t TC_X = 0, TC_D3 = 0, TC_H = 128, TC_ACC = 160, TC_ONE = 192;
constexpr int W16_W0HI = 0, W16_W0LO = 8192, W16_PW = 19456, W16_W2 = 23552;
constexpr int W16_B0T = 16384, W16_B1T = 16896;
constexpr int W16_B2T = 17408;
constexpr int W16_BYTES = 36864 + 2048 + 1024;
static_assert(W16_PW == W16_B2T + 2048 && W16_PW % 1024 == 0 && W16_W2 == W16_PW + 4096 && W16_BYTES == W16_W2 + 16384, "weight image layout");
constexpr int T16_A_CHUNK = 2080, T16_A_BYTES = 7 * T16_A_CHUNK + 2048;
static_assert(T16_A_BYTES <= W16_B1T, "the A tile overlays W0 hi / lo and conv0's bias tile only");
#ifdef OMK_T16_PIXEL_STENCIL
constexpr bool T16_ROWS = false;
#else
constexpr bool T16_ROWS = true;
#endif
// ... 131 lines not shown
    }
}
struct T16Req { uint32_t bA, wA, bB, wB, meta; };
struct T16ReqSpec { int wordA, wordB; uint32_t sA, sB, odd, turn; };
__device__ __forceinline__ T16ReqSpec t16_req_spec(int pc) {
    T16ReqSpec q;
    q.turn = pc >= 54;
    const int f0 = q.turn ? 0 : 3 * pc, cA = f0 >> 1, cB = cA + 1;
    q.wordA = cA >> 5; q.sA = cA & 31; q.wordB = cB >> 5; q.sB = cB & 31; q.odd = f0 & 1;
    return q;
}
__device__ __forceinline__ T16Req t16_req_load(const NNIn *row, const T16ReqSpec &q) {
    const uint32_t *rp = reinterpret_cast<const uint32_t *>(row);
    T16Req r;
    r.bA = rp[q.wordA]; r.wA = rp[3 + q.wordA]; r.bB = rp[q.wordB]; r.wB = rp[3 + q.wordB]; r.meta = rp[6];
    return r;
}
__device__ __forceinline__ uint32_t t16_req_combo(const T16Req &r, const T16ReqSpec &q) {
    const uint32_t bA = (r.bA >> q.sA) & 1u, wA = (r.wA >> q.sA) & 1u, bB = (r.bB >> q.sB) & 1u, wB = (r.wB >> q.sB) & 1u;
    const uint32_t persp = (r.meta ^ (r.meta >> 1)) & 1u;
    const bool e = (q.odd ^ persp) != 0;
    const uint32_t bY = q.odd ? bB : bA, wY = q.odd ? wB : wA;
    const uint32_t ch0 = e ? wA : bA, ch1 = e ? bY : wY, ch2 = e ? wB : bB;
    const uint32_t stones = ch0 | (ch1 << 1) | (ch2 << 2);
    return q.turn ? ((r.meta & 1u) ^ 1u) * 7u : stones;
}
__device__ __forceinline__ float2 t16_lds64(uint32_t a) {
    float2 v;
    asm volatile("ld.shared.v2.f32 {%0, %1}, [%2];" : "=f"(v.x), "=f"(v.y) : "r"(a));
    return v;
}
__device__ __forceinline__ void t16_sts32(uint32_t a, uint32_t v) { asm volatile("st.shared.u32 [%0], %1;" ::"r"(a), "r"(v) : "memory"); }
__device__ __forceinline__ void t16_row_stencil(uint32_t up, uint32_t mid, uint32_t dn, const float2 *w, uint32_t a_addr, int r0) {
    float2 o[kSide];
    constexpr uint32_t PX = T16_HSTRIDE * 4;
#pragma unroll
    for (int xi = 0; xi < kSide; ++xi) {
        const float2 i0 = t16_lds64(up + xi * PX), i1 = t16_lds64(mid + xi * PX), i2 = t16_lds64(dn + xi * PX);
        if (xi > 0) {
            o[xi - 1] = __ffma2_rn(i0, w[2], o[xi - 1]); o[xi - 1] = __ffma2_rn(i1, w[5], o[xi - 1]); o[xi - 1] = __ffma2_rn(i2, w[8], o[xi - 1]);
        }
        o[xi] = xi > 0 ? __ffma2_rn(i0, w[1], o[xi]) : __fmul2_rn(i0, w[1]);
        o[xi] = __ffma2_rn(i1, w[4], o[xi]); o[xi] = __ffma2_rn(i2, w[7], o[xi]);
        if (xi + 1 < kSide) {
            o[xi + 1] = __fmul2_rn(i0, w[0]);
            o[xi + 1] = __ffma2_rn(i1, w[3], o[xi + 1]); o[xi + 1] = __ffma2_rn(i2, w[6], o[xi + 1]);
        }
    }
#pragma unroll
    for (int xo = 0; xo < kSide; ++xo) {
        uint32_t hi, lo;
        split2_f16(o[xo].x, o[xo].y, hi, lo);
        const int R = r0 + xo;
        if (R >= 0 && R < 128) {
            t16_sts32(a_addr + (uint32_t)(xo * 16), hi);
            t16_sts32(a_addr + (uint32_t)(xo * 16 + 4 * T16_A_CHUNK), lo);
        }
    }
}
__device__ __forceinline__ int t16_chan(int h, int c) { return 32 * h + c + (c >= 32 ? 32 : 0); }
__device__ __forceinline__ void t16_issue_conv0(uint32_t tmem_base, uint32_t wb, uint32_t zero) {
    constexpr int K0 = 0, K1 = 8;
    const uint64_t bhi = desc_sw128(wb + W16_W0HI), blo = desc_sw128(wb + W16_W0LO);
    const uint32_t dcol = tmem_base + TC_ACC;
#pragma unroll
    for (int kk = K0; kk < K1; ++kk) {
        const uint64_t off = (uint64_t)(((kk >> 2) * 4096 + (kk & 3) * 32) >> 4);
        const uint32_t ahi = tmem_base + TC_X + 16u * kk;
        umma_f16_ts(dcol, ahi + 8u, bhi + off, T16_IDESC_N32, kk != 0);
        umma_f16_ts(dcol, ahi, blo + off, T16_IDESC_N32, 1u);
        umma_f16_ts(dcol, ahi, bhi + off, T16_IDESC_N32, 1u);
    }
    if (K1 == 8)
        umma_f16_ts(dcol, tmem_base + TC_ONE, desc_nosw(wb + W16_B0T, zero - (wb + W16_B0T), 128u), T16_IDESC_N32, 1u);
}
#define T16_HALF(call_0, call_1) do { if (half == 0) { call_0; } else { call_1; } } while (0)

template <bool STAMPS, bool BOARDS>
__global__ void __launch_bounds__(T16_THREADS, 2)
    k_tower16(const uint8_t *__restrict__ wimg, const __grid_constant__ Tower16Params P, const NNIn *__restrict__ nn_in,
              const float *__restrict__ images, const uint32_t *n_req, int max_rows, const __grid_constant__ CUtensorMap map_hi,
              const __grid_constant__ CUtensorMap map_lo, const float *__restrict__ pimg) {
    extern __shared__ uint8_t t16_smem_raw[];
    const int rows = __shfl_sync(0xffffffffu, (int)min(*n_req, (uint32_t)max_rows), 0);
    const int n_triples = (rows + 2) / 3, n_pairs = (int)gridDim.x >> 1, pair = (int)blockIdx.x >> 1;
    if (pair >= n_triples) return;
    const uint32_t rank = cluster_rank();
    const int t = threadIdx.x, warp = __shfl_sync(0xffffffffu, t >> 5, 0), lane = t & 31;
    const int q = warp & 3, half = warp >> 2;
    const int R = (int)rank * 128 + q * 32 + lane;
    const int j = R / kCells, p = R - j * kCells;
    const int slot = j - (int)rank;
    const bool in_tile = R < 3 * kCells;
    const bool band = j == 1 && (rank == 0 ? p >= 37 : p <= 56);
    const int unit = warp * 2 + (lane >> 4), cp = lane & 15;
    const bool has_unit = unit < (rank == 0 ? 15 : 13);
    const int uj = rank == 0 ? (unit >= 9 ? 1 : 0) : (unit < 4 ? 1 : 2);
    const int urow = rank == 0 ? (unit >= 9 ? unit - 9 : unit) : (unit < 4 ? unit + 5 : unit - 4);

    uint8_t *sm = t16_smem_raw + ((1024u - (smem_u32(t16_smem_raw) & 1023u)) & 1023u);
    const uint32_t sbase = smem_u32(sm);
    float *H0 = reinterpret_cast<float *>(sm + S16_H);
    float *T32 = reinterpret_cast<float *>(sm + S16_TAB);
    float *IMG = reinterpret_cast<float *>(sm + S16_IMG);
    float *T0 = IMG;
    uint32_t *TW = reinterpret_cast<uint32_t *>(sm + S16_H);
    const uint32_t bar_w0 = sbase + S16_BAR, bar_mma = sbase + S16_BAR + 16, bar_band = sbase + S16_BAR + 24,
                   bar_free = sbase + S16_BAR + 32, tmem_slot = sbase + S16_BAR + 40, bar_mma2 = sbase + S16_BAR + 48;
    const uint32_t peer_h0 = mapa(sbase + S16_H, rank ^ 1u);
    const uint32_t peer_band = mapa(bar_band, rank ^ 1u), peer_free = mapa(bar_free, rank ^ 1u);

    if (t == 0) {
        mbar_init(bar_w0, 1);
        mbar_init(bar_w0 + 8, 1);
        mbar_init(bar_mma, 8);
        mbar_init(bar_band, 1);
        mbar_init(bar_free, 1);
        mbar_init(bar_mma2, 1);
        mbar_fence_init();
    }
    for (int e = t; e < 2048 / 16; e += T16_THREADS) reinterpret_cast<uint4 *>(sm + S16_ZERO)[e] = make_uint4(0u, 0u, 0u, 0u);
    fence_proxy_async_smem();
    for (int e = BOARDS ? t : 8 * 64; e < 8 * 64; e += T16_THREADS) {
        const int combo = e >> 6, ch = (e & 63) * 2;
        const float v0 = (float)(combo & 1), v1 = (float)((combo >> 1) & 1), v2 = (float)(combo >> 2);
        float2 sv = __ffma2_rn(make_float2(v0, v0), make_float2(P.wstem[0][ch], P.wstem[0][ch + 1]),
                               make_float2(P.bstem[ch], P.bstem[ch + 1]));
        sv = __ffma2_rn(make_float2(v1, v1), make_float2(P.wstem[1][ch], P.wstem[1][ch + 1]), sv);
        sv = __ffma2_rn(make_float2(v2, v2), make_float2(P.wstem[2][ch], P.wstem[2][ch + 1]), sv);
        const float a0 = t16_lrelu(sv.x), a1 = t16_lrelu(sv.y);
        T32[combo * T16_TABSTRIDE + ch] = a0;
        T32[combo * T16_TABSTRIDE + ch + 1] = a1;
        uint32_t hi, lo;
        split2_f16(a0, a1, hi, lo);
        TW[combo * T16_TABSTRIDE + (ch >> 4) * 16 + ((ch & 15) >> 1)] = hi;
        TW[combo * T16_TABSTRIDE + (ch >> 4) * 16 + 8 + ((ch & 15) >> 1)] = lo;
    }
    if (warp == 1) tmem_alloc<1>(tmem_slot, T16_TMEM_COLS);
    fence_before();
    __syncthreads();
    cluster_sync_all();
    fence_after();
    uint32_t tmem_base;
    asm volatile("ld.shared.u32 %0, [%1];" : "=r"(tmem_base) : "r"(tmem_slot));
    tmem_base = __shfl_sync(0xffffffffu, tmem_base, 0);
    const uint32_t tlane = tmem_base + ((uint32_t)(q * 32) << 16);

    {
        uint32_t one8[8] = {0u, 0u, 0u, 0u, 0u, 0u, 0u, 0u};
        const __half2 o2 = __floats2half2_rn(T16_BIAS_ONE, T16_BIAS_ONE);
        one8[0] = *reinterpret_cast<const uint32_t *>(&o2);
        tmem_st8(tlane + TC_ONE, one8);
        tmem_wait_st();
    }
    uint32_t g = 0;
    uint32_t mma_uses = 0;
    auto issue_weights = [&](uint32_t gg) {
        const uint32_t buf = gg & 1u, bar = bar_w0 + 8 * buf;
        fence_proxy_async_smem();
        mbar_expect_tx(bar, (uint32_t)W16_BYTES);
        const uint8_t *src = wimg + (size_t)(gg % 3u) * W16_BYTES;
        for (int c = 0; c < W16_BYTES; c += W16_BYTES / 4) bulk_load(sbase + S16_W + buf * W16_BYTES + c, src + c, W16_BYTES / 4, bar);
    };
    if (t == 0) issue_weights(0);

    if constexpr (BOARDS) {
        if (warp == 0) {
            const uint4 *tw = reinterpret_cast<const uint4 *>(TW + min(lane, 7) * T16_TABSTRIDE);
#pragma unroll
            for (int c = 0; c < 8; ++c) {
                uint32_t w[16];
#pragma unroll
                for (int k = 0; k < 4; ++k) {
                    const uint4 v = tw[c * 4 + k];
                    w[4 * k + 0] = v.x; w[4 * k + 1] = v.y; w[4 * k + 2] = v.z; w[4 * k + 3] = v.w;
                }
                tmem_st16(tlane + TC_X + (uint32_t)(c * 16), w);
            }
            tmem_wait_st();
        }
        fence_before();
        __syncthreads();
        if (warp == 0) {
            if (elect_one()) {
                fence_after();
                mbar_wait(bar_w0, 0u);
                t16_issue_conv0(tmem_base, sbase + S16_W, sbase + S16_ZERO);
                umma_commit(bar_mma);
            }
        } else if (lane == 0) {
            fence_after();
            umma_commit(bar_mma);
        }
        T16_WAIT(bar_mma, mma_uses & 1u);
        ++mma_uses;
        fence_after();
        if (warp == 0) {
            float d[32], o[32];
            tmem_ld16(tlane + TC_ACC, d);
            tmem_ld16(tlane + TC_ACC + 16, d + 16);
            tmem_wait_ld();
            t16_lrelu_scaled16(P.blk[0].inv[0], d, o);
            t16_lrelu_scaled16(P.blk[0].inv[0], d + 16, o + 16);
            if (lane < 8) {
#pragma unroll
                for (int c = 0; c < 32; c += 4)
                    *reinterpret_cast<float4 *>(T0 + lane * T16_HSTRIDE + c) = make_float4(o[c], o[c + 1], o[c + 2], o[c + 3]);
            }
        }
        fence_before();
        __syncthreads();
    }

    const T16ReqSpec spec = t16_req_spec(in_tile ? p : 0);
    T16Req cur{};
    if constexpr (BOARDS) cur = t16_req_load(nn_in + min(pair * 3 + j, rows - 1), spec);
    int pos_iter = 0;
    for (int tr = pair; tr < n_triples; tr += n_pairs, ++pos_iter) {
        [[maybe_unused]] const bool dbg_on = blockIdx.x == 0 && pos_iter == 1;
        const int row = tr * 3 + j;
        const bool real = in_tile && row < rows;
        T16_STAMP(0);
        float x[64];
        [[maybe_unused]] uint32_t combo = 0;
        if constexpr (!BOARDS) {
            if (t < 243) {
                IMG[t] = images[(size_t)min(tr * 3 + 0, rows - 1) * 243 + t];
                IMG[243 + t] = images[(size_t)min(tr * 3 + 1, rows - 1) * 243 + t];
                IMG[486 + t] = images[(size_t)min(tr * 3 + 2, rows - 1) * 243 + t];
            }
            __syncthreads();
            const int pc = real ? p : 0;
            const float *im = IMG + (real ? j : 0) * 243;
            const float v0 = im[3 * pc], v1 = im[3 * pc + 1], v2 = im[3 * pc + 2];
            T16_HALF(t16_stem<0>(P, v0, v1, v2, x), t16_stem<1>(P, v0, v1, v2, x));
#pragma unroll
            for (int c = 0; c < 4; ++c) t16_store_group(tlane + TC_X + (uint32_t)t16_chan(half, c * 16), x + c * 16);
        } else {
            combo = t16_req_combo(cur, spec);
            if (tr + n_pairs < n_triples) cur = t16_req_load(nn_in + min((tr + n_pairs) * 3 + j, rows - 1), spec);
            const float4 *tx = reinterpret_cast<const float4 *>(T32 + combo * T16_TABSTRIDE + half * 32);
#pragma unroll
            for (int c = 0; c < 16; ++c) {
                const float4 v = tx[c + (c >= 8 ? 8 : 0)];
                x[4 * c + 0] = v.x; x[4 * c + 1] = v.y; x[4 * c + 2] = v.z; x[4 * c + 3] = v.w;
            }
        }
        if constexpr (!BOARDS) tmem_wait_st();
        T16_STAMP(1);

#pragma unroll 1
        for (int r = 0; r < 3; ++r, ++g) {
            const Tower16Block &B = P.blk[r];
            const uint32_t wb = sbase + S16_W + (g & 1u) * W16_BYTES;
            if (r == 0 && lane == 0) bulk_wait_read0();
            fence_before();
            __syncthreads();
            const bool table0 = BOARDS && r == 0;
            if (table0) {
                if (warp == 3 && lane == 0) {
                    issue_weights(g + 1);
                    mbar_expect_tx(bar_band, T16_BAND_BYTES);
                }
            } else {
                if (warp == 0) {
                    if (elect_one()) {
                        fence_after();
                        mbar_wait(bar_w0 + 8 * (g & 1u), (g >> 1) & 1u);
                        t16_issue_conv0(tmem_base, wb, sbase + S16_ZERO);
                        umma_commit(bar_mma);
                    }
                } else if (lane == 0) {
                    fence_after();
                    if (warp == 3) {
                        issue_weights(g + 1);
                        mbar_expect_tx(bar_band, T16_BAND_BYTES);
                    }
                    umma_commit(bar_mma);
                }
                T16_WAIT_MMA(bar_mma, mma_uses & 1u);
                ++mma_uses;
                fence_after();
            }
            T16_STAMP(2 + r * 8 + 0);
            {
                float d[16], o[16];
                if (table0) {
                    const float4 *t0 = reinterpret_cast<const float4 *>(T0 + combo * T16_HSTRIDE + half * 16);
#pragma unroll
                    for (int c = 0; c < 4; ++c) {
                        const float4 v = t0[c];
                        o[4 * c + 0] = v.x; o[4 * c + 1] = v.y; o[4 * c + 2] = v.z; o[4 * c + 3] = v.w;
                    }
                } else {
                    tmem_ld16(tlane + TC_ACC + half * 16, d);
                    tmem_wait_ld();
                    t16_lrelu_scaled16(B.inv[0], d, o);
                }
                if (in_tile) {
// ... 242 lines not shown
            pb[P16_INV + 0] = 1.0f / s0;
            pb[P16_INV + 1] = 1.0f / s1;
            pb[P16_INV + 2] = 1.0f / s2;
            pb[P16_INV + 3] = 0.0f;
        }
    }
    for (int i = tid; i < 384; i += nth) pimg[P16_WSTEM + i] = a.conv_w[i];
    for (int i = tid; i < 128; i += nth) pimg[P16_BSTEM + i] = a.conv_b[i];
}

bool tower16_prepare_weights(omk_ctx *c) {
    NetWeights &w = *c->model;
    if (!w.tower16_wimg) {
        TowerImages t;
        if (t.tower16_wimg.alloc(3 * W16_BYTES) != cudaSuccess || t.tower16_pimg.alloc(P16_FLOATS) != cudaSuccess ||
            t.tower16_absmax.alloc(18) != cudaSuccess)
            return false;
        static_cast<TowerImages &>(w) = std::move(t);
    }
    Tower16PackArgs a;
    a.conv_w = w.t[0];
    a.conv_b = w.t[1];
    for (int r = 0; r < 3; ++r) {
        const int b = 2 + 7 * r;
        a.w0[r] = w.t[b + 0]; a.b0[r] = w.t[b + 1]; a.dw[r] = w.t[b + 2]; a.pw[r] = w.t[b + 3];
        a.b1[r] = w.t[b + 4]; a.w2[r] = w.t[b + 5]; a.b2[r] = w.t[b + 6];
    }
    cudaMemsetAsync(w.tower16_absmax, 0, sizeof(uint32_t) * 18, c->stream);
    cudaMemsetAsync(w.tower16_wimg, 0, 3 * W16_BYTES, c->stream);
    k_tower16_absmax<<<18, 256, 0, c->stream>>>(a, w.tower16_absmax);
    k_tower16_pack<<<16, 256, 0, c->stream>>>(a, w.tower16_absmax, w.tower16_wimg, w.tower16_pimg);
    c->launches += 2;
    w.tower16_params_host.resize(sizeof(Tower16Params));
    if (cudaMemcpyAsync(w.tower16_params_host.data(), w.tower16_pimg, sizeof(Tower16Params), cudaMemcpyDeviceToHost, c->stream) != cudaSuccess) return false;
    if (cudaStreamSynchronize(c->stream) != cudaSuccess) return false;
    return true;
}

void tower16_read_timing(long long *out64) { cudaMemcpyFromSymbol(out64, g_t16_dbg, sizeof(long long) * 64); }

static int tower16_max_pairs(omk_ctx *c) {
    if (c->tower16_pairs > 0) return c->tower16_pairs;
    cudaLaunchConfig_t cfg{};
    cfg.gridDim = dim3(2 * 2 * c->n_sms);
    cfg.blockDim = dim3(T16_THREADS);
    cfg.dynamicSmemBytes = T16_SMEM_BYTES;
    cudaLaunchAttribute attr[1];
    attr[0].id = cudaLaunchAttributeClusterDimension;
    attr[0].val.clusterDim.x = 2;
    attr[0].val.clusterDim.y = 1;
    attr[0].val.clusterDim.z = 1;
    cfg.attrs = attr;
    cfg.numAttrs = 1;
    int n = c->n_sms;
    int api = 0;
    if (cudaOccupancyMaxActiveClusters(&api, k_tower16<false, true>, &cfg) != cudaSuccess) cudaGetLastError();
    if (getenv("OMK_DEBUG")) {
        int per_sm = -1;
        cudaOccupancyMaxActiveBlocksPerMultiprocessor(&per_sm, k_tower16<false, true>, T16_THREADS, T16_SMEM_BYTES);
        cudaFuncAttributes fa{};
        cudaFuncGetAttributes(&fa, k_tower16<false, true>);
        fprintf(stderr, "omok_b200: k_tower16 CTA pairs: %d (%d SMs); occupancy API: %d clusters, %d blocks/SM; regs %d, static smem %zu, max dyn smem %d, carveout %d\n",
                n, c->n_sms, api, per_sm, fa.numRegs, fa.sharedSizeBytes, fa.maxDynamicSharedSizeBytes, fa.preferredShmemCarveout);
    }
    if (const char *e = getenv("OMK_TOWER_PAIRS")) n = atoi(e) > 0 ? atoi(e) : n;
    c->tower16_pairs = n;
    return n;
}

bool launch_tower_f16(omk_ctx *c, const float *images_dev, int rows_bound) {
    static const bool stamps = getenv("OMK_TOWER_STAMPS") && atoi(getenv("OMK_TOWER_STAMPS")) != 0;
    const bool boards = images_dev == nullptr;
    auto kern = stamps ? (boards ? k_tower16<true, true> : k_tower16<true, false>) : (boards ? k_tower16<false, true> : k_tower16<false, false>);
    cudaFuncSetAttribute(kern, cudaFuncAttributeMaxDynamicSharedMemorySize, T16_SMEM_BYTES);
    cudaFuncSetAttribute(kern, cudaFuncAttributePreferredSharedMemoryCarveout, cudaSharedmemCarveoutMaxShared);
    const int triples = (rows_bound + 2) / 3;
    const int max_pairs = tower16_max_pairs(c);
    const int pairs = triples < max_pairs ? triples : max_pairs;
    cudaLaunchConfig_t cfg{};
    cfg.gridDim = dim3(2 * pairs);
    cfg.blockDim = dim3(T16_THREADS);
    cfg.dynamicSmemBytes = T16_SMEM_BYTES;
    cfg.stream = c->stream;
    cudaLaunchAttribute attr[1];
    attr[0].id = cudaLaunchAttributeClusterDimension;
    attr[0].val.clusterDim.x = 2;
    attr[0].val.clusterDim.y = 1;
    attr[0].val.clusterDim.z = 1;
    cfg.attrs = attr;
    cfg.numAttrs = 1;
    const NetWeights &m = *c->model;
    const uint8_t *wimg = m.tower16_wimg;
    if (m.tower16_params_host.empty()) return false;
    const Tower16Params &params = *reinterpret_cast<const Tower16Params *>(m.tower16_params_host.data());
    const NNIn *nn_in = c->ws.nn_in;
    const uint32_t *n_req = c->ws.n_req;
    const ActMaps &maps = c->ws.maps;
    const float *pimg = m.tower16_pimg;
    const cudaError_t e = cudaLaunchKernelEx(&cfg, kern, wimg, params, nn_in, images_dev, n_req, rows_bound, maps.tower_st_hi,
                                             maps.tower_st_lo, pimg);
    if (e != cudaSuccess) fprintf(stderr, "omok_b200: cudaLaunchKernelEx(k_tower16): %s\n", cudaGetErrorString(e));
    c->launches++;
    return e == cudaSuccess;
}

}
```

### omok-ai_b200/csrc/tree_kernels.cu

```cuda
#include "omk_internal.h"

namespace omk {

constexpr int kWarpsPerBlock = 4;
constexpr unsigned kFull = 0xffffffffu;

struct TreeArgs {
    TreeHdr *hdrs;
    uint8_t *nodes;
    int cap_nodes;
    const int32_t *ids;
    int id_base;
    int n;
    uint64_t seed;
    uint32_t *dev_error;
    unsigned long long *dev_sims;
    NNIn *nn_in;
    uint32_t *req_tree, *req_node;
    uint32_t *n_req;
    uint32_t *slot_base, *slot_count;
    const float *P, *V;
    int max_rows;
    int vloss;
};

__device__ __forceinline__ int tree_of(const TreeArgs &a, int slot) { return a.ids ? a.ids[slot] : slot + a.id_base; }
__device__ __forceinline__ uint8_t *tree_nodes_of(const TreeArgs &a, int tree) {
    return a.nodes + (size_t)tree * (size_t)a.cap_nodes * kNodeBytes;
}

__device__ __forceinline__ float dummy_prior(const NodeHdr &h, int a) {
    const uint32_t occ = sel3(h.black[0] | h.white[0], h.black[1] | h.white[1], h.black[2] | h.white[2], a >> 5);
    if ((occ >> (a & 31)) & 1u) return 0.0f;
    if (h.legal == 0) return 1.0f;
    return __fmul_rn(1.0f, __fdiv_rn(1.0f, (float)h.legal));
}

__device__ __forceinline__ float seq_sum81(const float v[3]) {
    float s = 0.0f;
#pragma unroll
    for (int j = 0; j < 3; ++j) {
        const int lim = j == 2 ? kCells - 64 : 32;
        for (int l = 0; l < lim; ++l) s = __fadd_rn(s, __shfl_sync(kFull, v[j], l));
    }
    return s;
}

__device__ __forceinline__ void backup_path(uint8_t *tn, const uint32_t *path, int depth, float v, uint32_t &root_n,
                                            float &root_w) {
    for (int d = depth - 1; d >= 0; --d) {
        uint8_t *pn = node_ptr(tn, path[d] >> 8);
        const int a = path[d] & 0xFF;
        node_edge_n(pn)[a] += 1u;
        node_edge_w(pn)[a] = __fadd_rn(node_edge_w(pn)[a], v);
        v = -v;
    }
    root_n += 1u;
    root_w = __fadd_rn(root_w, v);
}

__global__ void __launch_bounds__(kWarpsPerBlock * 32)
    k_new_games(TreeArgs a, const uint32_t *streams, const int8_t *only_if_terminal, const float *root_policy) {
    const int slot = blockIdx.x * kWarpsPerBlock + (threadIdx.x >> 5);
    const int lane = threadIdx.x & 31;
    if (slot >= a.n) return;
    const int tree = tree_of(a, slot);
    uint8_t *tn = tree_nodes_of(a, tree);
    if (only_if_terminal) {
        const int st = only_if_terminal[slot];
        if (st != kDraw && st != kBlackWin && st != kWhiteWin) {
            if (lane == 0) a.slot_count[slot] = 0;
            return;
        }
    }
    if (root_policy) {
        float *pol = node_policy(tn);
        for (int c = lane; c < kCells; c += 32) pol[c] = root_policy[c];
    }
    if (lane == 0) {
        TreeHdr th{};
        th.n_nodes = 1;
        th.root_n = 0;
        th.root_w = 0.0f;
        th.root_p = 1.0f;
        if (only_if_terminal) {
            const TreeHdr old = a.hdrs[tree];
            th.rng_counter = old.rng_counter;
            th.stream = old.stream;
            th.noise_epoch = old.noise_epoch;
        } else {
            th.rng_counter = 0;
            th.stream = streams ? streams[slot] : (uint32_t)tree;
            th.noise_epoch = 0;
        }
        a.hdrs[tree] = th;
        NodeHdr h{};
        h.parent = kNoNode;
        h.action = 0xFF;
        h.status = kInProgress;
        h.legal = kCells;
        h.turn = 0;
        h.has_policy = root_policy ? 1 : 0;
        store_hdr(tn, h);
        if (root_policy) {
            a.slot_count[slot] = 0;
        } else {
            const uint32_t row = atomicAdd(a.n_req, 1u);
            a.slot_base[slot] = row;
            a.slot_count[slot] = row < (uint32_t)a.max_rows ? 1 : 0;
            if (row < (uint32_t)a.max_rows) {
                NNIn in{};
                a.nn_in[row] = in;
                a.req_tree[row] = (uint32_t)tree;
                a.req_node[row] = 0;
            }
        }
    }
}

__global__ void __launch_bounds__(kWarpsPerBlock * 32) k_root_noise(TreeArgs a, float epsilon, float alpha) {
    const int slot = blockIdx.x * kWarpsPerBlock + (threadIdx.x >> 5);
    const int lane = threadIdx.x & 31;
    if (slot >= a.n) return;
    const int tree = tree_of(a, slot);
    uint8_t *tn = tree_nodes_of(a, tree);
    TreeHdr *th = &a.hdrs[tree];
    NodeHdr h = load_hdr(tn);
    float *pol = node_policy(tn);

    float p[3], nz[3];
#pragma unroll
    for (int j = 0; j < 3; ++j) {
        const int c = lane + 32 * j;
        p[j] = 0.0f;
        nz[j] = 0.0f;
        if (c < kCells) p[j] = h.has_policy ? pol[c] : dummy_prior(h, c);
    }
    if (epsilon != 0.0f) {
        const uint32_t epoch = th->noise_epoch;
        const uint32_t stream = th->stream;
#pragma unroll
        for (int j = 0; j < 3; ++j) {
            const int c = lane + 32 * j;
            if (c < kCells) nz[j] = noise_gamma_cell(a.seed, stream, epoch, c, alpha);
        }
        __syncwarp();
        const float s = seq_sum81(nz);
        const float inv = __fdiv_rn(1.0f, s);
#pragma unroll
        for (int j = 0; j < 3; ++j) nz[j] = __fmul_rn(nz[j], inv);
        if (lane == 0) th->noise_epoch = epoch + 1;
    }
    const float keep = __fsub_rn(1.0f, epsilon);
#pragma unroll
    for (int j = 0; j < 3; ++j) p[j] = __fadd_rn(__fmul_rn(keep, p[j]), __fmul_rn(epsilon, nz[j]));
    const float s = seq_sum81(p);
    const float inv = __fdiv_rn(1.0f, s);
#pragma unroll
    for (int j = 0; j < 3; ++j) {
        const int c = lane + 32 * j;
        if (c < kCells) pol[c] = __fmul_rn(p[j], inv);
    }
    if (lane == 0 && !h.has_policy) {
        h.has_policy = 1;
        store_hdr(tn, h);
    }
}

__global__ void __launch_bounds__(kWarpsPerBlock * 32) k_select_expand(TreeArgs a, int batch) {
    __shared__ uint32_t s_path[kWarpsPerBlock][kCells + 3];
    __shared__ uint16_t s_req[kWarpsPerBlock][kMaxBatchPerTree];
    const int wib = threadIdx.x >> 5;
    const int slot = blockIdx.x * kWarpsPerBlock + wib;
    const int lane = threadIdx.x & 31;
    if (slot >= a.n) return;
    const int tree = tree_of(a, slot);
    uint8_t *tn = tree_nodes_of(a, tree);
    TreeHdr *th = &a.hdrs[tree];
    uint32_t *path = s_path[wib];
    uint16_t *req = s_req[wib];

    uint32_t n_nodes = th->n_nodes;
    uint32_t root_n = th->root_n;
    float root_w = th->root_w;
    uint32_t rng_counter = th->rng_counter;
    const uint32_t stream = th->stream;
    uint32_t err = th->error;
    uint32_t sims = 0;
    int nreq = 0;

    bool restart = true;
    uint32_t x = 0;
    uint32_t cur_n = root_n;
    int depth = 0;
    NodeHdr h{};
    int it = 0;
    while (it < batch && !err) {
        if (restart) {
            x = 0;
            cur_n = root_n;
            depth = 0;
            h = load_hdr(tn);
            restart = false;
        }
        for (;;) {
            const int nch = popc81(h.cmask);
            if (nch != (int)h.legal || nch == 0) break;
            uint8_t *xn = node_ptr(tn, x);
            const uint32_t parent_n = cur_n > 1u ? cur_n : 1u;
            const float sq = __fsqrt_rn((float)parent_n);
            const uint32_t *en = node_edge_n(xn);
            const float *ew = node_edge_w(xn);
            const float *pol = node_policy(xn);
            const uint16_t *ch = node_child(xn);
            unsigned long long best = 0ull;
            uint32_t best_n = 0;
            int best_a = 0;
#pragma unroll
            for (int j = 0; j < 3; ++j) {
                const int c = lane + 32 * j;
                if (c < kCells && bit81(h.cmask, c)) {
                    const uint32_t n = en[c];
                    const float w = ew[c];
                    const float p = h.has_policy ? pol[c] : dummy_prior(h, c);
                    const float q = __fdiv_rn(w, __fadd_rn((float)n, kF32Eps));
                    const float bias = __fdiv_rn(sq, (float)(1u + n));
                    const float u = __fadd_rn(q, __fmul_rn(__fmul_rn(1.0f, p), bias));
                    const uint32_t okey = (uint32_t)total_order_key(u) ^ 0x80000000u;
                    const unsigned long long cand = ((unsigned long long)okey << 32) | (unsigned long long)(ch[c] + 1u);
                    if (cand > best) {
                        best = cand;
                        best_n = n;
                        best_a = c;
                    }
                }
            }
            unsigned long long wbest = best;
#pragma unroll
            for (int off = 16; off > 0; off >>= 1) {
                const unsigned long long o = __shfl_xor_sync(kFull, wbest, off);
                wbest = o > wbest ? o : wbest;
            }
            const int src = __ffs(__ballot_sync(kFull, best == wbest && best != 0ull)) - 1;
            best_n = __shfl_sync(kFull, best_n, src);
            best_a = __shfl_sync(kFull, best_a, src);
            if (lane == 0) path[depth] = (x << 8) | (uint32_t)best_a;
            ++depth;
            x = (uint32_t)(wbest & 0xFFFFFFFFull) - 1u;
            cur_n = best_n;
            h = load_hdr(node_ptr(tn, x));
        }
        __syncwarp();

        if (h.status != kInProgress) {
// ... 69 lines not shown
            if (lane < t_first) req[nreq + lane] = (uint16_t)id;
        }
#pragma unroll
        for (int k = 0; k < 3; ++k) {
            add[k] = __reduce_or_sync(kFull, add[k]);
            h.cmask[k] |= add[k];
        }
        if (lane < 3 && sel3(add[0], add[1], add[2], lane)) reinterpret_cast<uint32_t *>(xn)[6 + lane] = sel3(h.cmask[0], h.cmask[1], h.cmask[2], lane);
        if (accepted > 0) rng_counter = __shfl_sync(kFull, my_ctr, accepted - 1);
        n_nodes += (uint32_t)accepted;
        nreq += min(t_first, accepted);
        it += accepted;
        sims += (uint32_t)accepted;
        __syncwarp();
        if (term_accepted) {
            const int t_action = __shfl_sync(kFull, my_action, t_first);
            const bool t_five = __shfl_sync(kFull, (int)five, t_first) != 0;
            if (lane == 0) {
                path[depth] = (x << 8) | (uint32_t)t_action;
                backup_path(tn, path, depth + 1, t_five ? 1.0f : 0.0f, root_n, root_w);
            }
            restart = true;
        } else if (a.vloss && accepted == 1) {
            const int v_action = __shfl_sync(kFull, my_action, 0);
            if (lane == 0) {
                path[depth] = (x << 8) | (uint32_t)v_action;
                for (int d = depth; d >= 0; --d) {
                    uint8_t *pn = node_ptr(tn, path[d] >> 8);
                    const int pa = path[d] & 0xFF;
                    node_edge_n(pn)[pa] += 1u;
                    node_edge_w(pn)[pa] = __fsub_rn(node_edge_w(pn)[pa], 1.0f);
                }
                root_n += 1u;
            }
            restart = true;
        }
#ifdef OMK_NO_DESCENT_REUSE
        restart = true;
#endif
        root_n = __shfl_sync(kFull, root_n, 0);
        root_w = __shfl_sync(kFull, root_w, 0);
        __syncwarp();
    }

    uint32_t base = 0;
    if (lane == 0) base = nreq ? atomicAdd(a.n_req, (uint32_t)nreq) : 0u;
    base = __shfl_sync(kFull, base, 0);
    if (base + (uint32_t)nreq > (uint32_t)a.max_rows) {
        err = 1;
        nreq = 0;
    }
    __syncwarp();
    for (int i = lane; i < nreq; i += 32) {
        const uint32_t id = req[i];
        const NodeHdr r = load_hdr(node_ptr(tn, id));
        NNIn in;
        in.black[0] = r.black[0]; in.black[1] = r.black[1]; in.black[2] = r.black[2];
        in.white[0] = r.white[0]; in.white[1] = r.white[1]; in.white[2] = r.white[2];
        in.meta = r.turn;
        in.pad = 0;
        a.nn_in[base + i] = in;
        a.req_tree[base + i] = (uint32_t)tree;
        a.req_node[base + i] = id;
    }
    if (lane == 0) {
        a.slot_base[slot] = base;
        a.slot_count[slot] = (uint32_t)nreq;
        th->n_nodes = n_nodes;
        th->root_n = root_n;
        th->root_w = root_w;
        th->rng_counter = rng_counter;
        if (err) {
            th->error = err;
            atomicOr(a.dev_error, 1u);
        }
        atomicAdd(a.dev_sims, (unsigned long long)sims);
    }
}

__global__ void __launch_bounds__(kWarpsPerBlock * 32) k_apply(TreeArgs a, int mode) {
    constexpr int kChunk = 16;
    __shared__ float s_p[kWarpsPerBlock][kChunk][kCells];
    __shared__ uint32_t s_meta[kWarpsPerBlock][kChunk][4];
    const int wib = threadIdx.x >> 5;
    const int slot = blockIdx.x * kWarpsPerBlock + wib;
    const int lane = threadIdx.x & 31;
    if (slot >= a.n) return;
    const int tree = tree_of(a, slot);
    uint8_t *tn = tree_nodes_of(a, tree);
    TreeHdr *th = &a.hdrs[tree];
    const uint32_t base = a.slot_base[slot];
    const int cnt = (int)a.slot_count[slot];
    if (cnt == 0) return;
    uint32_t root_n = th->root_n;
    float root_w = th->root_w;
    uint32_t root_occ[3] = {0u, 0u, 0u};
    if (mode == kApplyEnsure) {
        const NodeHdr root_h = load_hdr(tn);
#pragma unroll
        for (int k = 0; k < 3; ++k) root_occ[k] = root_h.black[k] | root_h.white[k];
    }
    float(*sp)[kCells] = s_p[wib];
    uint32_t(*meta)[4] = s_meta[wib];

    for (int c0 = 0; c0 < cnt; c0 += kChunk) {
        const int m = min(kChunk, cnt - c0);
        const uint32_t row0 = base + (uint32_t)c0;
        uint32_t my_id = 0, my_action = 0;
        float my_v = 0.0f;
        uint32_t my_occ[3] = {0u, 0u, 0u};
        if (lane < m) {
            my_id = a.req_node[row0 + lane];
            if (mode == kApplySearch) my_v = -a.V[row0 + lane];
            const NodeHdr h = load_hdr(node_ptr(tn, my_id));
#pragma unroll
            for (int k = 0; k < 3; ++k) my_occ[k] = h.black[k] | h.white[k];
            my_action = h.action;
            meta[lane][0] = my_id;
            meta[lane][1] = h.parent | (h.action << 16);
            meta[lane][2] = h.legal | (h.turn << 8) | (1u << 16);
            meta[lane][3] = __float_as_uint(my_v);
        }
#pragma unroll 8
        for (int i = 0; i < m; ++i) {
            const float *Prow = a.P + (size_t)(row0 + i) * kRow;
            float pv[3];
#pragma unroll
            for (int j = 0; j < 3; ++j) {
                const int c = lane + 32 * j;
                pv[j] = c < kCells ? Prow[c] : 0.0f;
            }
            const uint32_t o0 = __shfl_sync(kFull, my_occ[0], i), o1 = __shfl_sync(kFull, my_occ[1], i), o2 = __shfl_sync(kFull, my_occ[2], i);
            const int act_i = (int)__shfl_sync(kFull, my_action, i);
#pragma unroll
            for (int j = 0; j < 3; ++j) {
                const int c = lane + 32 * j;
                if (c < kCells) {
                    float v = pv[j];
                    if (mode == kApplySearch) {
                        const uint32_t occ = sel3(o0, o1, o2, j);
                        if ((occ >> (c & 31)) & 1u) v = 0.0f;
                    } else if (mode == kApplyEnsure) {
                        const uint32_t occ = sel3(root_occ[0], root_occ[1], root_occ[2], j);
                        if (c == act_i || ((occ >> (c & 31)) & 1u)) v = 0.0f;
                    }
                    sp[i][c] = v;
                }
            }
        }
        __syncwarp();
        float inv = 0.0f;
        bool scale = false;
        if (mode != kApplyNewGame && lane < m) {
            float sum = 0.0f;
#pragma unroll 9
            for (int c = 0; c < kCells; ++c) sum = __fadd_rn(sum, sp[lane][c]);
            scale = kF32Eps <= sum;
            if (scale) inv = __fdiv_rn(1.0f, sum);
        }
#pragma unroll 4
        for (int i = 0; i < m; ++i) {
            const float inv_i = __shfl_sync(kFull, inv, i);
            const bool scale_i = __shfl_sync(kFull, (int)scale, i) != 0;
            const uint32_t id = __shfl_sync(kFull, my_id, i);
            float *pol = node_policy(node_ptr(tn, id));
#pragma unroll
// ... 374 lines not shown
        __syncwarp();
        if (lane == 0) {
            const uint32_t np = id == c ? kNoNode : (uint32_t)remap[hs.parent];
            reinterpret_cast<uint32_t *>(dst)[9] = np | (hs.action << 16) | (hs.status << 24);
        }
        if (has_children) {
            uint16_t *ch = node_child(dst);
#pragma unroll
            for (int j = 0; j < 3; ++j) {
                const int k = lane + 32 * j;
                if (k < kCells && bit81(hs.cmask, k)) ch[k] = remap[ch[k]];
            }
        }
        __syncwarp();
    }
    if (lane == 0) {
        th->n_nodes = kept;
        th->root_n = new_root_n;
        th->root_w = new_root_w;
        th->root_p = new_root_p;
    }
}

__global__ void k_root_children(TreeArgs a, int tree, int32_t *out_actions, unsigned long long *out_n, float *out_w,
                                float *out_p, int32_t *out_len, float *out_policy, uint32_t *out_misc) {
    uint8_t *tn = tree_nodes_of(a, tree);
    const TreeHdr *th = &a.hdrs[tree];
    const NodeHdr h = load_hdr(tn);
    if (threadIdx.x == 0) {
        int len = 0;
        long long last_id = -1;
        for (;;) {
            int best_a = -1;
            long long best_id = 1ll << 40;
            for (int c = 0; c < kCells; ++c) {
                if (!bit81(h.cmask, c)) continue;
                const long long cid = node_child(tn)[c];
                if (cid > last_id && cid < best_id) {
                    best_id = cid;
                    best_a = c;
                }
            }
            if (best_a < 0) break;
            last_id = best_id;
            out_actions[len] = best_a;
            out_n[len] = node_edge_n(tn)[best_a];
            out_w[len] = node_edge_w(tn)[best_a];
            out_p[len] = h.has_policy ? node_policy(tn)[best_a] : dummy_prior(h, best_a);
            ++len;
        }
        *out_len = len;
        out_misc[0] = th->root_n;
        out_misc[1] = __float_as_uint(th->root_w);
        out_misc[2] = __float_as_uint(th->root_p);
        out_misc[3] = h.status;
        out_misc[4] = th->n_nodes;
        out_misc[5] = th->rng_counter;
        out_misc[6] = h.turn | (h.legal << 8);
        out_misc[7] = th->error;
        for (int k = 0; k < 3; ++k) {
            out_misc[8 + k] = h.black[k];
            out_misc[11 + k] = h.white[k];
        }
    }
    for (int c = threadIdx.x; c < kCells; c += blockDim.x)
        out_policy[c] = h.has_policy ? node_policy(tn)[c] : dummy_prior(h, c);
}

__global__ void k_pool_get_envs(TreeArgs a, uint8_t *boards, uint8_t *turns, uint16_t *legal, int8_t *status) {
    const int slot = blockIdx.x;
    if (slot >= a.n) return;
    const NodeHdr h = load_hdr(tree_nodes_of(a, tree_of(a, slot)));
    if (boards)
        for (int c = threadIdx.x; c < kCells; c += blockDim.x)
            boards[(size_t)slot * kCells + c] = bit81(h.black, c) ? 1 : (bit81(h.white, c) ? 2 : 0);
    if (threadIdx.x == 0) {
        if (turns) turns[slot] = (uint8_t)h.turn;
        if (legal) legal[slot] = (uint16_t)h.legal;
        if (status) status[slot] = (int8_t)h.status;
    }
}

__global__ void k_eval_hash(const NNIn *in, const uint32_t *n_req, float *P, float *V, int max_rows) {
    const uint32_t rows = min(*n_req, (uint32_t)max_rows);
    const uint32_t idx = blockIdx.x * blockDim.x + threadIdx.x;
    const uint32_t row = idx / kRow, c = idx % kRow;
    if (row >= rows) return;
    const NNIn r = in[row];
    const uint64_t hsh = hash_board(r.black, r.white, r.meta & 1u, (r.meta >> 1) & 1u);
    if (c < (uint32_t)kCells) P[(size_t)row * kRow + c] = hash_policy(hsh, (int)c);
    if (c == (uint32_t)kCells) V[row] = hash_value(hsh);
}

__global__ void k_reset_requests(uint32_t *n_req, unsigned long long *dev_sims) {
    atomicAdd(&dev_sims[1], (unsigned long long)*n_req);
    *n_req = 0;
}

__global__ void k_sp_prepare(int g0, int n, const int32_t *ply, int threshold, float temperature, int32_t *mover, int32_t *other,
                             uint8_t *modes, float *temps) {
    const int g = g0 + blockIdx.x * blockDim.x + threadIdx.x;
    if (g >= g0 + n) return;
    const int p = ply[g];
    mover[g] = 2 * g + (p & 1);
    other[g] = 2 * g + 1 - (p & 1);
    modes[g] = p < threshold ? OMK_SAMPLE_BOLTZMANN : OMK_SAMPLE_BEST;
    temps[g] = temperature;
}

__global__ void k_sp_record(TreeArgs a, const int32_t *actions, const float *policy_in, uint8_t *boards_out,
                            float *policy_out, int32_t *actions_out) {
    const int g = blockIdx.x;
    if (g >= a.n) return;
    const int tree = tree_of(a, g);
    const NodeHdr h = load_hdr(tree_nodes_of(a, tree));
    for (int c = threadIdx.x; c < kCells; c += blockDim.x) {
        boards_out[(size_t)g * kCells + c] = bit81(h.black, c) ? 1 : (bit81(h.white, c) ? 2 : 0);
        policy_out[(size_t)g * kCells + c] = policy_in[(size_t)g * kCells + c];
    }
    if (threadIdx.x == 0) actions_out[g] = actions[g];
}

__global__ void k_sp_advance(int g0, int n, int32_t *ply, const int8_t *status, unsigned long long *counters, uint32_t *dev_error) {
    const int g = g0 + blockIdx.x * blockDim.x + threadIdx.x;
    if (g >= g0 + n) return;
    const int st = status[g];
    if (st == kDraw || st == kBlackWin || st == kWhiteWin) {
        ply[g] = 0;
        atomicAdd(&counters[0], 1ull);
    } else if (st == kInProgress) {
        ply[g] += 1;
    } else {
        atomicOr(dev_error, 4u);
    }
}

static TreeArgs make_args(omk_ctx *c, const int32_t *ids_dev, int n) {
    TreeArgs a{};
    a.hdrs = c->tree_hdrs;
    a.nodes = c->tree_nodes;
    a.cap_nodes = c->cap_nodes;
    a.ids = ids_dev;
    a.id_base = ids_dev ? 0 : c->id_base;
    a.n = n;
    a.seed = c->seed;
    a.dev_error = c->dev_error;
    a.dev_sims = c->dev_sims;
    a.nn_in = c->ws.nn_in;
    a.req_tree = c->ws.req_tree;
    a.req_node = c->ws.req_node;
    a.n_req = c->ws.n_req;
    a.slot_base = c->ws.slot_base;
    a.slot_count = c->ws.slot_count;
    a.P = c->ws.P;
    a.V = c->ws.V;
    a.max_rows = c->ws.max_rows;
    a.vloss = c->virtual_loss;
    return a;
}
static inline int warp_grid(int n) { return (n + kWarpsPerBlock - 1) / kWarpsPerBlock; }

void launch_reset_requests(omk_ctx *c) {
    k_reset_requests<<<1, 1, 0, c->stream>>>(c->ws.n_req, c->dev_sims);
    c->launches++;
}
void launch_new_games(omk_ctx *c, const int32_t *ids_dev, int n, const uint32_t *streams_dev,
                      const int8_t *only_if_terminal, const float *root_policy) {
    if (n <= 0) return;
    k_new_games<<<warp_grid(n), kWarpsPerBlock * 32, 0, c->stream>>>(make_args(c, ids_dev, n), streams_dev,
                                                                       only_if_terminal, root_policy);
    c->launches++;
}
void launch_sp_prepare(omk_ctx *c, int g0, int n, int32_t *mover, int32_t *other, uint8_t *modes, float *temps) {
    k_sp_prepare<<<(n + 127) / 128, 128, 0, c->stream>>>(g0, n, c->sp_ply, c->sp_cfg.temperature_threshold,
                                                          c->sp_cfg.temperature, mover, other, modes, temps);
    c->launches++;
}
void launch_sp_record(omk_ctx *c, int n, const int32_t *mover, const int32_t *actions, const float *policy_in,
                      uint8_t *boards_out, float *policy_out, int32_t *actions_out) {
    k_sp_record<<<n, 96, 0, c->stream>>>(make_args(c, mover, n), actions, policy_in, boards_out, policy_out, actions_out);
    c->launches++;
}
void launch_sp_advance(omk_ctx *c, int g0, int n, const int8_t *status, unsigned long long *counters) {
    k_sp_advance<<<(n + 127) / 128, 128, 0, c->stream>>>(g0, n, c->sp_ply, status, counters, c->dev_error);
    c->launches++;
}
void launch_root_noise(omk_ctx *c, const int32_t *ids_dev, int n, float epsilon, float alpha) {
    if (n <= 0) return;
    k_root_noise<<<warp_grid(n), kWarpsPerBlock * 32, 0, c->stream>>>(make_args(c, ids_dev, n), epsilon, alpha);
    c->launches++;
}
void launch_select_expand(omk_ctx *c, const int32_t *ids_dev, int n, int batch) {
    if (n <= 0) return;
    k_select_expand<<<warp_grid(n), kWarpsPerBlock * 32, 0, c->stream>>>(make_args(c, ids_dev, n), batch);
    c->launches++;
}
void launch_apply(omk_ctx *c, const int32_t *ids_dev, int n, int mode) {
    if (n <= 0) return;
    k_apply<<<warp_grid(n), kWarpsPerBlock * 32, 0, c->stream>>>(make_args(c, ids_dev, n), mode);
    c->launches++;
}
void launch_sample(omk_ctx *c, const int32_t *ids_dev, int n, const uint8_t *modes_dev, const float *temps_dev,
                   int32_t *actions_dev, float *policy_dev, uint8_t *valid_dev) {
    if (n <= 0) return;
    k_sample<<<warp_grid(n), kWarpsPerBlock * 32, 0, c->stream>>>(make_args(c, ids_dev, n), modes_dev, temps_dev,
                                                                    actions_dev, policy_dev, valid_dev);
    c->launches++;
}
void launch_ensure_prepare(omk_ctx *c, const int32_t *ids_dev, const int32_t *actions_dev, int n) {
    if (n <= 0) return;
    k_ensure_prepare<<<warp_grid(n), kWarpsPerBlock * 32, 0, c->stream>>>(make_args(c, ids_dev, n), actions_dev);
    c->launches++;
}
void launch_play(omk_ctx *c, const int32_t *ids_dev, const int32_t *actions_dev, int n, int8_t *status_dev) {
    if (n <= 0) return;
    k_play<<<warp_grid(n), kWarpsPerBlock * 32, 0, c->stream>>>(make_args(c, ids_dev, n), actions_dev, status_dev,
                                                                  c->remap);
    c->launches++;
}
void launch_root_children(omk_ctx *c, int tree, int32_t *actions_dev, unsigned long long *n_dev, float *w_dev,
                          float *p_dev, int32_t *len_dev, float *policy_dev, uint32_t *misc_dev) {
    k_root_children<<<1, 96, 0, c->stream>>>(make_args(c, nullptr, 1), tree, actions_dev, n_dev, w_dev, p_dev, len_dev,
                                              policy_dev, misc_dev);
    c->launches++;
}
void launch_pool_get_envs(omk_ctx *c, const int32_t *ids_dev, int n, uint8_t *boards_dev, uint8_t *turns_dev,
                          uint16_t *legal_dev, int8_t *status_dev) {
    if (n <= 0) return;
    k_pool_get_envs<<<n, 96, 0, c->stream>>>(make_args(c, ids_dev, n), boards_dev, turns_dev, legal_dev, status_dev);
    c->launches++;
}
void launch_eval_hash(omk_ctx *c, int rows_bound) {
    const int threads = 192;
    if (rows_bound > c->ws.max_rows) rows_bound = c->ws.max_rows;
    if (rows_bound <= 0) return;
    const long long total = (long long)rows_bound * kRow;
    k_eval_hash<<<(unsigned)((total + threads - 1) / threads), threads, 0, c->stream>>>(c->ws.nn_in, c->ws.n_req, c->ws.P,
                                                                                         c->ws.V, rows_bound);
    c->launches++;
}

}
```

### shims/omok-b200-sys/src/lib.rs

```rust
#![allow(non_camel_case_types)]
use std::ffi::CStr;
use std::os::raw::{c_char, c_void};
use std::sync::{Mutex, OnceLock};

pub const OMK_CELLS: usize = 81;
pub const OMK_NONE: i8 = -1;
pub const OMK_OK: i32 = 0;
pub const OMK_ERR_INVALID: i32 = -1;
pub const OMK_ERR_CUDA: i32 = -2;
pub const OMK_ERR_CAPACITY: i32 = -3;
pub const OMK_ERR_STATE: i32 = -4;
pub const OMK_ERR_NUMERIC: i32 = -5;
pub const OMK_EVAL_NET: i32 = 0;
pub const OMK_EVAL_HASH: i32 = 1;
pub const OMK_SAMPLE_BEST: u8 = 0;
pub const OMK_SAMPLE_BOLTZMANN: u8 = 1;
pub const OMK_TURN_MODE_PLAYER: i32 = 0;
pub const OMK_TURN_MODE_OPPONENT: i32 = 1;
pub const OMK_NET_TENSORS: usize = 31;
pub const OMK_K_COUNT: usize = 8;

#[repr(C)]
pub struct omk_ctx {
    _private: [u8; 0],
}

#[repr(C)]
#[derive(Clone, Copy, Debug)]
pub struct omk_selfplay_config {
    pub n_games: i32,
    pub count: i32,
    pub batch_size: i32,
    pub epsilon: f32,
    pub alpha: f32,
    pub temperature: f32,
    pub temperature_threshold: i32,
    pub evaluator: i32,
}

#[repr(C)]
#[derive(Clone, Copy, Debug, Default)]
pub struct omk_selfplay_stats {
    pub simulations: i64,
    pub positions: i64,
    pub nn_evals: i64,
    pub games_finished: i64,
    pub h2d_bytes: i64,
    pub d2h_bytes: i64,
    pub gpu_ms: f32,
    pub kind_ms: [f32; OMK_K_COUNT],
    pub kind_launches: [i64; OMK_K_COUNT],
}

extern "C" {
    pub fn omk_last_error() -> *const c_char;
    pub fn omk_version() -> i32;
    pub fn omk_ctx_create(device: i32, capacity_envs: i32, capacity_trees: i32, capacity_nodes: i32, seed: u64, out: *mut *mut omk_ctx) -> i32;
    pub fn omk_ctx_destroy(ctx: *mut omk_ctx) -> i32;
    pub fn omk_ctx_synchronize(ctx: *mut omk_ctx) -> i32;
    pub fn omk_ctx_stream(ctx: *mut omk_ctx) -> *mut c_void;
    pub fn omk_ctx_launch_count(ctx: *mut omk_ctx) -> i64;
    pub fn omk_ctx_transfer_bytes(ctx: *mut omk_ctx, out_h2d: *mut i64, out_d2h: *mut i64) -> i32;
    pub fn omk_net_load_params(ctx: *mut omk_ctx, tensors: *const *const f32, lens: *const i64) -> i32;
    pub fn omk_net_get_params(ctx: *mut omk_ctx, tensors: *const *mut f32, lens: *const i64) -> i32;
    pub fn omk_net_init_random(ctx: *mut omk_ctx, seed: u64) -> i32;
    pub fn omk_net_eval(ctx: *mut omk_ctx, boards: *const u8, turns: *const u8, n: i32, mode: i32, out_p: *mut f32, out_v: *mut f32) -> i32;
    pub fn omk_train_step(ctx: *mut omk_ctx, images: *const f32, pi: *const f32, z: *const f32, n: i32, out_losses: *mut f32) -> i32;
    pub fn omk_train_backward(ctx: *mut omk_ctx, images: *const f32, pi: *const f32, z: *const f32, n: i32, out_grads_device: *mut *mut c_void, out_count: *mut i64) -> i32;
    pub fn omk_train_apply(ctx: *mut omk_ctx, out_losses: *mut f32) -> i32;
    pub fn omk_train_get_grads(ctx: *mut omk_ctx, tensors: *const *mut f32, lens: *const i64) -> i32;
    pub fn omk_train_reset_optimizer(ctx: *mut omk_ctx) -> i32;
    pub fn omk_train_comm_unique_id(ctx: *mut omk_ctx, out_id: *mut u8) -> i32;
    pub fn omk_train_comm_init(ctx: *mut omk_ctx, id: *const u8, nranks: i32, rank: i32) -> i32;
    pub fn omk_train_comm_destroy(ctx: *mut omk_ctx) -> i32;
    pub fn omk_net_eval_images(ctx: *mut omk_ctx, images: *const f32, n: i32, out_p: *mut f32, out_v: *mut f32) -> i32;
    pub fn omk_debug_set_fc0_mode(ctx: *mut omk_ctx, mode: i32) -> i32;
    pub fn omk_debug_set_tower_mode(ctx: *mut omk_ctx, mode: i32) -> i32;
    pub fn omk_debug_set_fc0_chunk(ctx: *mut omk_ctx, k_blocks: i32) -> i32;
    pub fn omk_debug_set_fc0_balance(ctx: *mut omk_ctx, on: i32) -> i32;
    pub fn omk_debug_tower_timing(ctx: *mut omk_ctx, out64: *mut i64) -> i32;
    pub fn omk_debug_get_buffer(ctx: *mut omk_ctx, which: i32, out: *mut f32, count: i64) -> i32;
    pub fn omk_debug_set_lane_min_trees(ctx: *mut omk_ctx, min_trees: i32) -> i32;
    pub fn omk_env_reset(ctx: *mut omk_ctx, ids: *const i32, n: i32) -> i32;
    pub fn omk_env_step(ctx: *mut omk_ctx, ids: *const i32, actions: *const u8, n: i32, out_status: *mut i8, out_legal: *mut u32) -> i32;
    pub fn omk_env_step_device(ctx: *mut omk_ctx, actions_device: *const u8, n: i32, out_status_device: *mut i8, out_legal_device: *mut u32) -> i32;
    pub fn omk_env_get(ctx: *mut omk_ctx, ids: *const i32, n: i32, out_boards: *mut u8, out_turns: *mut u8, out_legal_counts: *mut u16) -> i32;
    pub fn omk_env_set(ctx: *mut omk_ctx, ids: *const i32, n: i32, boards: *const u8, turns: *const u8) -> i32;
    pub fn omk_env_encode(ctx: *mut omk_ctx, ids: *const i32, n: i32, mode: i32, out: *mut f32) -> i32;
    pub fn omk_env_random_playout(ctx: *mut omk_ctx, n: i32, plies: i32, out_actions: *mut u8, out_status: *mut i8) -> i32;
    pub fn omk_pool_new_games(ctx: *mut omk_ctx, ids: *const i32, n: i32, streams: *const u32, evaluator: i32) -> i32;
    pub fn omk_pool_search(ctx: *mut omk_ctx, ids: *const i32, n: i32, count: i32, batch_size: i32, epsilon: f32, alpha: f32, evaluator: i32) -> i32;
    pub fn omk_search_set_virtual_loss(ctx: *mut omk_ctx, enabled: i32) -> i32;
    pub fn omk_pool_sample(ctx: *mut omk_ctx, ids: *const i32, n: i32, modes: *const u8, temperatures: *const f32, out_actions: *mut i32, out_policy: *mut f32) -> i32;
    pub fn omk_pool_policy(ctx: *mut omk_ctx, ids: *const i32, n: i32, out_policy: *mut f32, out_valid: *mut u8) -> i32;
    pub fn omk_pool_ensure_action(ctx: *mut omk_ctx, ids: *const i32, actions: *const i32, n: i32, evaluator: i32) -> i32;
    pub fn omk_pool_play(ctx: *mut omk_ctx, ids: *const i32, actions: *const i32, n: i32, out_status: *mut i8) -> i32;
    pub fn omk_pool_get_env(ctx: *mut omk_ctx, id: i32, out_board: *mut u8, out_turn: *mut u8, out_legal_count: *mut u16) -> i32;
    pub fn omk_pool_get_envs(ctx: *mut omk_ctx, ids: *const i32, n: i32, out_boards: *mut u8, out_turns: *mut u8, out_legal_counts: *mut u16, out_status: *mut i8) -> i32;
    pub fn omk_pool_root_stats(ctx: *mut omk_ctx, id: i32, out_n: *mut u64, out_w: *mut f32, out_p: *mut f32, out_status: *mut i32, out_policy: *mut f32) -> i32;
    pub fn omk_pool_root_children(ctx: *mut omk_ctx, id: i32, out_actions: *mut i32, out_n: *mut u64, out_w: *mut f32, out_p: *mut f32, out_len: *mut i32) -> i32;
    pub fn omk_pool_tree_info(ctx: *mut omk_ctx, id: i32, out_nodes: *mut i32, out_rng_counter: *mut u32) -> i32;
    pub fn omk_selfplay_begin(ctx: *mut omk_ctx, cfg: *const omk_selfplay_config) -> i32;
    pub fn omk_selfplay_run(ctx: *mut omk_ctx, plies: i32, profile: i32, out_boards: *mut u8, out_policy: *mut f32, out_status: *mut i8, out_actions: *mut i32, stats: *mut omk_selfplay_stats) -> i32;
    pub fn omk_replay_reset(ctx: *mut omk_ctx, capacity: i64) -> i32;
    pub fn omk_replay_info(ctx: *mut omk_ctx, out_len: *mut i64, out_rows_added: *mut i64, out_episodes: *mut i64) -> i32;
    pub fn omk_replay_get(ctx: *mut omk_ctx, rows: *const i64, n: i32, out_boards: *mut u8, out_turns: *mut u8, out_policy: *mut f32, out_z: *mut f32) -> i32;
    pub fn omk_train_replay(ctx: *mut omk_ctx, seed: u64, first_step: i64, steps: i32, n: i32, out_losses: *mut f32, out_rows: *mut i64) -> i32;
    pub fn omk_naive_move(ctx: *mut omk_ctx, boards: *const u8, turns: *const u8, n: i32, seed: u64, streams: *const u32, out_actions: *mut i32, out_forced: *mut u8) -> i32;
    pub fn omk_eval_naive(ctx: *mut omk_ctx, episodes: i32, first_tree: i32, count: i32, batch_size: i32, epsilon: f32, alpha: f32, evaluator: i32, seed: u64, out_result: *mut i32, out_moves: *mut i8, out_status: *mut i8, out_stats: *mut i64, out_gpu_ms: *mut f32) -> i32;
    pub fn omk_opponent_load_params(ctx: *mut omk_ctx, tensors: *const *const f32, lens: *const i64) -> i32;
    pub fn omk_opponent_from_net(ctx: *mut omk_ctx) -> i32;
    pub fn omk_opponent_eval(ctx: *mut omk_ctx, boards: *const u8, turns: *const u8, n: i32, mode: i32, out_p: *mut f32, out_v: *mut f32) -> i32;
    pub fn omk_match(ctx: *mut omk_ctx, pairs: i32, first_tree: i32, count: i32, batch_size: i32, epsilon: f32, alpha: f32, evaluator: i32, out_result: *mut i32, out_moves: *mut i8, out_status: *mut i8, out_stats: *mut i64, out_gpu_ms: *mut f32) -> i32;
}

pub fn last_error() -> String {
    unsafe { CStr::from_ptr(omk_last_error()).to_string_lossy().into_owned() }
}

pub struct Context {
    raw: *mut omk_ctx,
    free_envs: Vec<i32>,
    free_trees: Vec<i32>,
}
unsafe impl Send for Context {}

static CTX: OnceLock<Mutex<Context>> = OnceLock::new();

fn env_or<T: std::str::FromStr>(name: &str, default: T) -> T {
    std::env::var(name).ok().and_then(|v| v.parse().ok()).unwrap_or(default)
}

impl Context {
    fn create() -> Context {
        let (device, envs, trees, nodes, seed) = (
            env_or("OMOK_B200_DEVICE", 0i32),
            env_or("OMOK_B200_ENVS", 65536i32),
            env_or("OMOK_B200_TREES", 4096i32),
            env_or("OMOK_B200_NODES", 4096i32),
            env_or("OMOK_B200_SEED", 0u64),
        );
        let mut raw = std::ptr::null_mut();
        let rc = unsafe { omk_ctx_create(device, envs, trees, nodes, seed, &mut raw) };
        assert!(rc == OMK_OK, "omk_ctx_create: {}", last_error());
        Context { raw, free_envs: (0..envs).rev().collect(), free_trees: (0..trees).rev().collect() }
    }
    pub fn raw(&self) -> *mut omk_ctx {
        self.raw
    }
    pub fn take_env(&mut self) -> i32 {
        self.free_envs.pop().expect("env pool exhausted: raise OMOK_B200_ENVS")
    }
    pub fn give_env(&mut self, slot: i32) {
        self.free_envs.push(slot)
    }
    pub fn take_tree(&mut self) -> i32 {
        self.free_trees.pop().expect("tree pool exhausted: raise OMOK_B200_TREES")
    }
    pub fn give_tree(&mut self, slot: i32) {
        self.free_trees.push(slot)
    }
}

pub fn with<R>(f: impl FnOnce(&mut Context) -> R) -> R {
    let m = CTX.get_or_init(|| Mutex::new(Context::create()));
// ... 12 lines not shown
```

Baseline: 17.30 million.

## Chain MCTS and network kernels with programmatic dependent launch and weight prefetch

Launches the tree kernels, tower, FC layers, heads, reduce and reset kernels with the programmatic stream serialization attribute, and each kernel now waits on griddepcontrol.wait before reading upstream data. The FC kernel issues TMA prefetches of the weight tiles for the first stages before the wait, and the tower does its setup before it. The row-count early exit moves after the wait, so idle blocks drain their prefilled barriers. The goal is to hide launch latency and weight-load time across the many small dependent kernels in each search step. The cost is added complexity in barrier accounting, and idle blocks now stay resident longer.

```diff
diff --git a/include/omok_b200.h b/include/omok_b200.h
--- a/include/omok_b200.h
+++ b/include/omok_b200.h
@@ -71,6 +71,7 @@
 OMK_API int32_t omk_debug_tower_timing(omk_ctx *ctx, int64_t *out64);
 OMK_API int32_t omk_debug_get_buffer(omk_ctx *ctx, int32_t which, float *out, int64_t count);
 OMK_API int32_t omk_debug_set_lane_min_trees(omk_ctx *ctx, int32_t min_trees);
+OMK_API int32_t omk_debug_set_pdl(omk_ctx *ctx, int32_t on);
 
 OMK_API int32_t omk_env_reset(omk_ctx *ctx, const int32_t *ids, int32_t n);
 OMK_API int32_t omk_env_step(omk_ctx *ctx, const int32_t *ids, const uint8_t *actions, int32_t n, int8_t *out_status,
diff --git a/omok-ai_b200/binding.py b/omok-ai_b200/binding.py
--- a/omok-ai_b200/binding.py
+++ b/omok-ai_b200/binding.py
@@ -110,6 +110,7 @@
     L.omk_debug_set_fc0_chunk.argtypes = [vp, i32]
     L.omk_debug_set_fc0_balance.argtypes = [vp, i32]
     L.omk_debug_set_lane_min_trees.argtypes = [vp, i32]
+    L.omk_debug_set_pdl.argtypes = [vp, i32]
     L.omk_debug_get_buffer.argtypes = [vp, i32, vp, i64]
     L.omk_debug_tower_timing.argtypes = [vp, vp]
     L.omk_env_reset.argtypes = [vp, vp, i32]
@@ -298,6 +299,9 @@
     def debug_set_lane_min_trees(self, min_trees: int):
         self._check(self.L.omk_debug_set_lane_min_trees(self.h, min_trees))
 
+    def debug_set_pdl(self, on: bool):
+        self._check(self.L.omk_debug_set_pdl(self.h, 1 if on else 0))
+
     def debug_tower_timing(self):
         out = np.zeros(64, dtype=np.int64)
         self._check(self.L.omk_debug_tower_timing(self.h, _ptr(out)))
diff --git a/omok-ai_b200/csrc/fc_f16.cu b/omok-ai_b200/csrc/fc_f16.cu
--- a/omok-ai_b200/csrc/fc_f16.cu
+++ b/omok-ai_b200/csrc/fc_f16.cu
@@ -72,7 +72,6 @@
     constexpr int NCHUNK = NKB / CHUNK;
     const int kb_base = SPLITK ? (int)blockIdx.z * F_SPLITK_KB : 0;
     extern __shared__ uint8_t smem_raw[];
-    const int rows = (int)min(*n_req, (uint32_t)max_rows);
     uint32_t rank = 0;
     int m0, n0;
     [[maybe_unused]] int role = 0, n_seq = NCHUNK, u0 = 0;
@@ -97,11 +96,9 @@
         const int pair = tile >> 1;
         m0 = pair * 256 + (int)rank * F_BM;
         n0 = (tile & 1) * BN;
-        if (role != 2 && pair * 256 >= rows) return;
     } else {
         m0 = blockIdx.y * F_BM;
         n0 = blockIdx.x * BN;
-        if (m0 >= rows) return;
     }
     const bool leader = rank == 0;
 
@@ -133,8 +130,27 @@
     fence_after();
     uint32_t tmem_base;
     asm volatile("ld.shared.u32 %0, [%1];" : "=r"(tmem_base) : "r"(tmem_slot));
-
-    if (warp == 0) {
+    constexpr int kPrefill = PAIR ? 0 : (NKB < Cfg::kStages ? NKB : Cfg::kStages);
+    if (warp == 0 && lane == 0) {
+        for (int s = 0; s < kPrefill; ++s) {
+            const uint32_t st = base + s * Cfg::kStageBytes, bar = full0 + 8 * s;
+            mbar_expect_tx_only(bar, 2 * Cfg::kBBytes);
+            tma_load_2d(st + 2 * F_A_BYTES, &map_b_hi, bar, (kb_base + s) * F_BK, n0);
+            tma_load_2d(st + 2 * F_A_BYTES + Cfg::kBBytes, &map_b_lo, bar, (kb_base + s) * F_BK, n0);
+        }
+    }
+    pdl_wait();
+    const int rows = (int)min(*n_req, (uint32_t)max_rows);
+    const bool idle = PAIR ? role != 2 && (tile >> 1) * 256 >= rows : m0 >= rows;
+
+    if (idle) {
+        if (warp == 0 && lane == 0) {
+            for (int s = 0; s < kPrefill; ++s) {
+                mbar_arrive(full0 + 8 * s);
+                mbar_wait(full0 + 8 * s, 0u);
+            }
+        }
+    } else if (warp == 0) {
         if (lane == 0) {
             if constexpr (PAIR) {
                 int it = 0;
@@ -169,11 +185,14 @@
                 if constexpr (PAIR) {
                 } else {
                     const uint32_t bar = full0 + 8 * s;
-                    mbar_expect_tx(bar, Cfg::kStageBytes);
+                    const bool prefilled = kb < kPrefill;
+                    mbar_expect_tx(bar, prefilled ? 2 * F_A_BYTES : Cfg::kStageBytes);
                     tma_load_2d(st, &map_a_hi, bar, (kb_base + kb) * F_BK, m0);
                     tma_load_2d(st + F_A_BYTES, &map_a_lo, bar, (kb_base + kb) * F_BK, m0);
-                    tma_load_2d(st + 2 * F_A_BYTES, &map_b_hi, bar, (kb_base + kb) * F_BK, n0);
-                    tma_load_2d(st + 2 * F_A_BYTES + Cfg::kBBytes, &map_b_lo, bar, (kb_base + kb) * F_BK, n0);
+                    if (!prefilled) {
+                        tma_load_2d(st + 2 * F_A_BYTES, &map_b_hi, bar, (kb_base + kb) * F_BK, n0);
+                        tma_load_2d(st + 2 * F_A_BYTES + Cfg::kBBytes, &map_b_lo, bar, (kb_base + kb) * F_BK, n0);
+                    }
                 }
             }
         }
@@ -361,6 +380,7 @@
 __global__ void k_fc0_reduce(const float *__restrict__ partial, int nchunks, int ws_rows, const float *__restrict__ bias,
                              const float *__restrict__ inv_scale_p, __half *__restrict__ C_hi, __half *__restrict__ C_lo,
                              const uint32_t *n_req, int max_rows) {
+    pdl_wait();
     const int rows = (int)min(*n_req, (uint32_t)max_rows);
     const int idx = blockIdx.x * blockDim.x + threadIdx.x;
     const int row = idx >> 6, j = (idx & 63) * 8;
@@ -559,20 +579,20 @@
             using Cfg = FcCfg<false, 128>;
             auto sk = fine ? k_fc16<F_K0, F_CHUNK0_FINE, false, 128, false, true> : k_fc16<F_K0, F_CHUNK0, false, 128, false, true>;
             cudaFuncSetAttribute(sk, cudaFuncAttributeMaxDynamicSharedMemorySize, Cfg::kSmemBytes);
-            sk<<<dim3(F_N / 128, mt, F_K0 / F_BK / F_SPLITK_KB), Cfg::kThreads, Cfg::kSmemBytes, c->stream>>>(
-                am->map0_a_hi, am->map0_a_lo, m.map0_b_hi, m.map0_b_lo, m.t[24], m.fc_inv_scale, partial, nullptr,
-                nullptr, c->ws.n_req, rows_bound, nullptr, nullptr, nullptr, FcBal{});
+            launch_chain(c, sk, dim3(F_N / 128, mt, F_K0 / F_BK / F_SPLITK_KB), Cfg::kThreads, Cfg::kSmemBytes, am->map0_a_hi,
+                         am->map0_a_lo, m.map0_b_hi, m.map0_b_lo, m.t[24], m.fc_inv_scale, partial, nullptr, nullptr,
+                         c->ws.n_req, rows_bound, nullptr, nullptr, nullptr, FcBal{});
         } else {
             using Cfg = FcCfg<false, 256>;
             auto sk = fine ? k_fc16<F_K0, F_CHUNK0_FINE, false, 256, false, true> : k_fc16<F_K0, F_CHUNK0, false, 256, false, true>;
             cudaFuncSetAttribute(sk, cudaFuncAttributeMaxDynamicSharedMemorySize, Cfg::kSmemBytes);
-            sk<<<dim3(F_N / F_BN, mt, F_K0 / F_BK / F_SPLITK_KB), Cfg::kThreads, Cfg::kSmemBytes, c->stream>>>(
-                am->map0_a_hi, am->map0_a_lo, m.map0s_b_hi, m.map0s_b_lo, m.t[24], m.fc_inv_scale, partial, nullptr,
-                nullptr, c->ws.n_req, rows_bound, nullptr, nullptr, nullptr, FcBal{});
-        }
-        k_fc0_reduce<<<(rows_bound * 64 + 255) / 256, 256, 0, c->stream>>>(partial, kChunks, ws_rows, m.t[24],
-                                                                            m.fc_inv_scale, c->ws.act1_h16, c->ws.act1_l16,
-                                                                            c->ws.n_req, rows_bound);
+            launch_chain(c, sk, dim3(F_N / F_BN, mt, F_K0 / F_BK / F_SPLITK_KB), Cfg::kThreads, Cfg::kSmemBytes, am->map0_a_hi,
+                         am->map0_a_lo, m.map0s_b_hi, m.map0s_b_lo, m.t[24], m.fc_inv_scale, partial, nullptr, nullptr,
+                         c->ws.n_req, rows_bound, nullptr, nullptr, nullptr, FcBal{});
+        }
+        launch_chain(c, k_fc0_reduce, dim3((rows_bound * 64 + 255) / 256), dim3(256), 0, partial, kChunks, ws_rows,
+                     (const float *)m.t[24], (const float *)m.fc_inv_scale, (__half *)c->ws.act1_h16, (__half *)c->ws.act1_l16,
+                     (const uint32_t *)c->ws.n_req, rows_bound);
         c->launches += 2;
         return check_launch("fc0 (fp16 split, split-K)");
     }
@@ -584,13 +604,14 @@
     cfg.blockDim = dim3(FcCfg<true, 256>::kThreads);
     cfg.dynamicSmemBytes = FcCfg<true, 256>::kSmemBytes;
     cfg.stream = c->stream;
-    cudaLaunchAttribute attr[1];
+    cudaLaunchAttribute attr[2];
     attr[0].id = cudaLaunchAttributeClusterDimension;
     attr[0].val.clusterDim.x = 2;
     attr[0].val.clusterDim.y = 1;
     attr[0].val.clusterDim.z = 1;
+    attr[1] = pdl_attr(c);
     cfg.attrs = attr;
-    cfg.numAttrs = 1;
+    cfg.numAttrs = 2;
     const float *bias_p = m.t[24];
     const float *inv_p = m.fc_inv_scale;
     float *c_f32 = nullptr;
@@ -645,9 +666,9 @@
     auto kern = k_fc16<F_K1, F_CHUNK1, false>;
     cudaFuncSetAttribute(kern, cudaFuncAttributeMaxDynamicSharedMemorySize, Cfg::kSmemBytes);
     const int mt = (rows_bound + F_BM - 1) / F_BM;
-    kern<<<dim3(F_N / F_BN, mt), Cfg::kThreads, Cfg::kSmemBytes, c->stream>>>(
-        am->map1_a_hi, am->map1_a_lo, m.map1_b_hi, m.map1_b_lo, m.t[26], m.fc_inv_scale + 1, nullptr, c->ws.act2_h16,
-        c->ws.act2_l16, c->ws.n_req, rows_bound, nullptr, nullptr, nullptr, FcBal{});
+    launch_chain(c, kern, dim3(F_N / F_BN, mt), Cfg::kThreads, Cfg::kSmemBytes, am->map1_a_hi, am->map1_a_lo, m.map1_b_hi,
+                 m.map1_b_lo, m.t[26], m.fc_inv_scale + 1, nullptr, c->ws.act2_h16, c->ws.act2_l16, c->ws.n_req, rows_bound,
+                 nullptr, nullptr, nullptr, FcBal{});
     c->launches++;
     return check_launch("fc1 (fp16 split)");
 }
@@ -660,9 +681,9 @@
     auto kern = k_fc16<F_K1, F_CHUNKH, false, 128, true>;
     cudaFuncSetAttribute(kern, cudaFuncAttributeMaxDynamicSharedMemorySize, Cfg::kSmemBytes);
     const int mt = (rows_bound + F_BM - 1) / F_BM;
-    kern<<<dim3(1, mt), Cfg::kThreads, Cfg::kSmemBytes, c->stream>>>(
-        am->map2_a_hi, am->map2_a_lo, m.map2_b_hi, m.map2_b_lo, m.heads_b, m.fc_inv_scale + 2, nullptr, nullptr, nullptr,
-        c->ws.n_req, rows_bound, c->ws.P, c->ws.V, c->dev_error, FcBal{});
+    launch_chain(c, kern, dim3(1, mt), Cfg::kThreads, Cfg::kSmemBytes, am->map2_a_hi, am->map2_a_lo, m.map2_b_hi, m.map2_b_lo,
+                 m.heads_b, m.fc_inv_scale + 2, nullptr, nullptr, nullptr, c->ws.n_req, rows_bound, c->ws.P, c->ws.V,
+                 c->dev_error, FcBal{});
     c->launches++;
     return check_launch("heads (fp16 split)");
 }
diff --git a/omok-ai_b200/csrc/omk_api.cu b/omok-ai_b200/csrc/omk_api.cu
--- a/omok-ai_b200/csrc/omk_api.cu
+++ b/omok-ai_b200/csrc/omk_api.cu
@@ -577,6 +577,11 @@
     c->lane_min_trees = min_trees;
     return OMK_OK;
 }
+extern "C" int32_t omk_debug_set_pdl(omk_ctx *c, int32_t on) {
+    if (on != 0 && on != 1) return fail(OMK_ERR_INVALID, "pdl must be 0 (plain stream order) or 1 (programmatic dependent launch)");
+    c->pdl = on;
+    return OMK_OK;
+}
 extern "C" int32_t omk_debug_tower_timing(omk_ctx *c, int64_t *out64) {
     CK(cudaSetDevice(c->device));
     CK(cudaStreamSynchronize(c->stream));
diff --git a/omok-ai_b200/csrc/omk_internal.h b/omok-ai_b200/csrc/omk_internal.h
--- a/omok-ai_b200/csrc/omk_internal.h
+++ b/omok-ai_b200/csrc/omk_internal.h
@@ -221,6 +221,7 @@
     int train_n = 0;
     bool net_pack_dirty = false;
     int tower_mode = 1;
+    int pdl = 1;
 
     omk_selfplay_config sp_cfg{};
     bool sp_active = false;
@@ -238,6 +239,25 @@
 };
 
 namespace omk {
+
+inline cudaLaunchAttribute pdl_attr(const omk_ctx *c) {
+    cudaLaunchAttribute a{};
+    a.id = cudaLaunchAttributeProgrammaticStreamSerialization;
+    a.val.programmaticStreamSerializationAllowed = c->pdl ? 1 : 0;
+    return a;
+}
+template <typename... KArgs, typename... Args>
+cudaError_t launch_chain(const omk_ctx *c, void (*kern)(KArgs...), dim3 grid, dim3 block, size_t smem, Args &&...args) {
+    cudaLaunchConfig_t cfg{};
+    cfg.gridDim = grid;
+    cfg.blockDim = block;
+    cfg.dynamicSmemBytes = smem;
+    cfg.stream = c->stream;
+    cudaLaunchAttribute attr[1] = {pdl_attr(c)};
+    cfg.attrs = attr;
+    cfg.numAttrs = 1;
+    return cudaLaunchKernelEx(&cfg, kern, std::forward<Args>(args)...);
+}
 
 void launch_env_reset(omk_ctx *c, const int32_t *ids_dev, int n);
 void launch_env_step(omk_ctx *c, const int32_t *ids_dev, const uint8_t *actions_dev, int n, int8_t *status_dev,
diff --git a/omok-ai_b200/csrc/tc_ptx.cuh b/omok-ai_b200/csrc/tc_ptx.cuh
--- a/omok-ai_b200/csrc/tc_ptx.cuh
+++ b/omok-ai_b200/csrc/tc_ptx.cuh
@@ -18,6 +18,9 @@
 }
 __device__ __forceinline__ void mbar_arrive(uint32_t bar) {
     asm volatile("mbarrier.arrive.shared::cta.b64 _, [%0];" ::"r"(bar) : "memory");
+}
+__device__ __forceinline__ void mbar_expect_tx_only(uint32_t bar, uint32_t bytes) {
+    asm volatile("mbarrier.expect_tx.relaxed.cta.shared::cta.b64 [%0], %1;" ::"r"(bar), "r"(bytes) : "memory");
 }
 __device__ __forceinline__ void mbar_arrive_cluster(uint32_t cluster_bar) {
     asm volatile("mbarrier.arrive.release.cluster.shared::cluster.b64 _, [%0];" ::"r"(cluster_bar) : "memory");
@@ -62,6 +65,8 @@
     cluster_arrive();
     cluster_wait();
 }
+
+__device__ __forceinline__ void pdl_wait() { asm volatile("griddepcontrol.wait;" ::: "memory"); }
 
 __device__ __forceinline__ void bulk_load(uint32_t dst, const void *src, uint32_t bytes, uint32_t bar) {
     asm volatile("cp.async.bulk.shared::cluster.global.mbarrier::complete_tx::bytes [%0], [%1], %2, [%3];"
diff --git a/omok-ai_b200/csrc/tower_f16.cu b/omok-ai_b200/csrc/tower_f16.cu
--- a/omok-ai_b200/csrc/tower_f16.cu
+++ b/omok-ai_b200/csrc/tower_f16.cu
@@ -237,9 +237,7 @@
               const float *__restrict__ images, const uint32_t *n_req, int max_rows, const __grid_constant__ CUtensorMap map_hi,
               const __grid_constant__ CUtensorMap map_lo, const float *__restrict__ pimg) {
     extern __shared__ uint8_t t16_smem_raw[];
-    const int rows = __shfl_sync(0xffffffffu, (int)min(*n_req, (uint32_t)max_rows), 0);
-    const int n_triples = (rows + 2) / 3, n_pairs = (int)gridDim.x >> 1, pair = (int)blockIdx.x >> 1;
-    if (pair >= n_triples) return;
+    const int n_pairs = (int)gridDim.x >> 1, pair = (int)blockIdx.x >> 1;
     const uint32_t rank = cluster_rank();
     const int t = threadIdx.x, warp = __shfl_sync(0xffffffffu, t >> 5, 0), lane = t & 31;
     const int q = warp & 3, half = warp >> 2;
@@ -367,9 +365,13 @@
         __syncthreads();
     }
 
+    pdl_wait();
+    const int rows = __shfl_sync(0xffffffffu, (int)min(*n_req, (uint32_t)max_rows), 0);
+    const int n_triples = (rows + 2) / 3;
+
     const T16ReqSpec spec = t16_req_spec(in_tile ? p : 0);
     T16Req cur{};
-    if constexpr (BOARDS) cur = t16_req_load(nn_in + min(pair * 3 + j, rows - 1), spec);
+    if (BOARDS && pair < n_triples) cur = t16_req_load(nn_in + min(pair * 3 + j, rows - 1), spec);
     int pos_iter = 0;
     for (int tr = pair; tr < n_triples; tr += n_pairs, ++pos_iter) {
         [[maybe_unused]] const bool dbg_on = blockIdx.x == 0 && pos_iter == 1;
@@ -778,13 +780,14 @@
     cfg.blockDim = dim3(T16_THREADS);
     cfg.dynamicSmemBytes = T16_SMEM_BYTES;
     cfg.stream = c->stream;
-    cudaLaunchAttribute attr[1];
+    cudaLaunchAttribute attr[2];
     attr[0].id = cudaLaunchAttributeClusterDimension;
     attr[0].val.clusterDim.x = 2;
     attr[0].val.clusterDim.y = 1;
     attr[0].val.clusterDim.z = 1;
+    attr[1] = pdl_attr(c);
     cfg.attrs = attr;
-    cfg.numAttrs = 1;
+    cfg.numAttrs = 2;
     const NetWeights &m = *c->model;
     const uint8_t *wimg = m.tower16_wimg;
     if (m.tower16_params_host.empty()) return false;
diff --git a/omok-ai_b200/csrc/tree_kernels.cu b/omok-ai_b200/csrc/tree_kernels.cu
--- a/omok-ai_b200/csrc/tree_kernels.cu
+++ b/omok-ai_b200/csrc/tree_kernels.cu
@@ -1,6 +1,9 @@
 #include "omk_internal.h"
+#include "tc_ptx.cuh"
 
 namespace omk {
+
+using tc::pdl_wait;
 
 constexpr int kWarpsPerBlock = 4;
 constexpr unsigned kFull = 0xffffffffu;
@@ -119,6 +122,7 @@
 }
 
 __global__ void __launch_bounds__(kWarpsPerBlock * 32) k_root_noise(TreeArgs a, float epsilon, float alpha) {
+    pdl_wait();
     const int slot = blockIdx.x * kWarpsPerBlock + (threadIdx.x >> 5);
     const int lane = threadIdx.x & 31;
     if (slot >= a.n) return;
@@ -170,6 +174,7 @@
 __global__ void __launch_bounds__(kWarpsPerBlock * 32) k_select_expand(TreeArgs a, int batch) {
     __shared__ uint32_t s_path[kWarpsPerBlock][kCells + 3];
     __shared__ uint16_t s_req[kWarpsPerBlock][kMaxBatchPerTree];
+    pdl_wait();
     const int wib = threadIdx.x >> 5;
     const int slot = blockIdx.x * kWarpsPerBlock + wib;
     const int lane = threadIdx.x & 31;
@@ -405,6 +410,7 @@
     constexpr int kChunk = 16;
     __shared__ float s_p[kWarpsPerBlock][kChunk][kCells];
     __shared__ uint32_t s_meta[kWarpsPerBlock][kChunk][4];
+    pdl_wait();
     const int wib = threadIdx.x >> 5;
     const int slot = blockIdx.x * kWarpsPerBlock + wib;
     const int lane = threadIdx.x & 31;
@@ -945,6 +951,7 @@
 }
 
 __global__ void k_eval_hash(const NNIn *in, const uint32_t *n_req, float *P, float *V, int max_rows) {
+    pdl_wait();
     const uint32_t rows = min(*n_req, (uint32_t)max_rows);
     const uint32_t idx = blockIdx.x * blockDim.x + threadIdx.x;
     const uint32_t row = idx / kRow, c = idx % kRow;
@@ -956,6 +963,7 @@
 }
 
 __global__ void k_reset_requests(uint32_t *n_req, unsigned long long *dev_sims) {
+    pdl_wait();
     atomicAdd(&dev_sims[1], (unsigned long long)*n_req);
     *n_req = 0;
 }
@@ -1024,7 +1032,7 @@
 static inline int warp_grid(int n) { return (n + kWarpsPerBlock - 1) / kWarpsPerBlock; }
 
 void launch_reset_requests(omk_ctx *c) {
-    k_reset_requests<<<1, 1, 0, c->stream>>>(c->ws.n_req, c->dev_sims);
+    launch_chain(c, k_reset_requests, dim3(1), dim3(1), 0, (uint32_t *)c->ws.n_req, (unsigned long long *)c->dev_sims);
     c->launches++;
 }
 void launch_new_games(omk_ctx *c, const int32_t *ids_dev, int n, const uint32_t *streams_dev,
@@ -1050,17 +1058,17 @@
 }
 void launch_root_noise(omk_ctx *c, const int32_t *ids_dev, int n, float epsilon, float alpha) {
     if (n <= 0) return;
-    k_root_noise<<<warp_grid(n), kWarpsPerBlock * 32, 0, c->stream>>>(make_args(c, ids_dev, n), epsilon, alpha);
+    launch_chain(c, k_root_noise, dim3(warp_grid(n)), dim3(kWarpsPerBlock * 32), 0, make_args(c, ids_dev, n), epsilon, alpha);
     c->launches++;
 }
 void launch_select_expand(omk_ctx *c, const int32_t *ids_dev, int n, int batch) {
     if (n <= 0) return;
-    k_select_expand<<<warp_grid(n), kWarpsPerBlock * 32, 0, c->stream>>>(make_args(c, ids_dev, n), batch);
+    launch_chain(c, k_select_expand, dim3(warp_grid(n)), dim3(kWarpsPerBlock * 32), 0, make_args(c, ids_dev, n), batch);
     c->launches++;
 }
 void launch_apply(omk_ctx *c, const int32_t *ids_dev, int n, int mode) {
     if (n <= 0) return;
-    k_apply<<<warp_grid(n), kWarpsPerBlock * 32, 0, c->stream>>>(make_args(c, ids_dev, n), mode);
+    launch_chain(c, k_apply, dim3(warp_grid(n)), dim3(kWarpsPerBlock * 32), 0, make_args(c, ids_dev, n), mode);
     c->launches++;
 }
 void launch_sample(omk_ctx *c, const int32_t *ids_dev, int n, const uint8_t *modes_dev, const float *temps_dev,
@@ -1098,9 +1106,9 @@
     if (rows_bound > c->ws.max_rows) rows_bound = c->ws.max_rows;
     if (rows_bound <= 0) return;
     const long long total = (long long)rows_bound * kRow;
-    k_eval_hash<<<(unsigned)((total + threads - 1) / threads), threads, 0, c->stream>>>(c->ws.nn_in, c->ws.n_req, c->ws.P,
-                                                                                         c->ws.V, rows_bound);
-    c->launches++;
-}
-
-}
+    launch_chain(c, k_eval_hash, dim3((unsigned)((total + threads - 1) / threads)), dim3(threads), 0, (const NNIn *)c->ws.nn_in,
+                 (const uint32_t *)c->ws.n_req, (float *)c->ws.P, (float *)c->ws.V, rows_bound);
+    c->launches++;
+}
+
+}
diff --git a/shims/omok-b200-sys/src/lib.rs b/shims/omok-b200-sys/src/lib.rs
--- a/shims/omok-b200-sys/src/lib.rs
+++ b/shims/omok-b200-sys/src/lib.rs
@@ -81,6 +81,7 @@
     pub fn omk_debug_tower_timing(ctx: *mut omk_ctx, out64: *mut i64) -> i32;
     pub fn omk_debug_get_buffer(ctx: *mut omk_ctx, which: i32, out: *mut f32, count: i64) -> i32;
     pub fn omk_debug_set_lane_min_trees(ctx: *mut omk_ctx, min_trees: i32) -> i32;
+    pub fn omk_debug_set_pdl(ctx: *mut omk_ctx, on: i32) -> i32;
     pub fn omk_env_reset(ctx: *mut omk_ctx, ids: *const i32, n: i32) -> i32;
     pub fn omk_env_step(ctx: *mut omk_ctx, ids: *const i32, actions: *const u8, n: i32, out_status: *mut i8, out_legal: *mut u32) -> i32;
     pub fn omk_env_step_device(ctx: *mut omk_ctx, actions_device: *const u8, n: i32, out_status_device: *mut i8, out_legal_device: *mut u32) -> i32;
```

Result: no change. 17.38 million, median of 6 (+0.5%).
